# lucidrains/vector-quantize-pytorch

Hardware: NVIDIA H100
Metric: vectors quantized/sec at dim=256, codebook=1024; indices bit-exact vs ref (higher is better)
Workload: dtype bf16

## Files before the change

vector_quantize_pytorch_b200/csrc/ptx.cuh:

```cuda
#pragma once
#include <cuda.h>
#include <cuda_runtime.h>
#include <stdint.h>

namespace vqb {

__device__ __forceinline__ uint32_t smem_u32(const void* p) {
  return static_cast<uint32_t>(__cvta_generic_to_shared(p));
}

__device__ __forceinline__ void mbar_init(uint32_t bar, uint32_t count) {
  asm volatile("mbarrier.init.shared::cta.b64 [%0], %1;" ::"r"(bar), "r"(count));
}
__device__ __forceinline__ void fence_barrier_init() {
  asm volatile("fence.mbarrier_init.release.cluster;" ::: "memory");
}
__device__ __forceinline__ void mbar_arrive(uint32_t bar) {
  asm volatile("mbarrier.arrive.shared::cta.b64 _, [%0];" ::"r"(bar) : "memory");
}
__device__ __forceinline__ void mbar_arrive_expect_tx(uint32_t bar, uint32_t bytes) {
  asm volatile("mbarrier.arrive.expect_tx.shared::cta.b64 _, [%0], %1;" ::"r"(bar), "r"(bytes) : "memory");
}
__device__ __forceinline__ bool mbar_try_wait(uint32_t bar, uint32_t parity) {
  uint32_t ok;
  asm volatile(
      "{\n"
      ".reg .pred p;\n"
      "mbarrier.try_wait.parity.shared::cta.b64 p, [%1], %2;\n"
      "selp.u32 %0, 1, 0, p;\n"
      "}\n"
      : "=r"(ok)
      : "r"(bar), "r"(parity)
      : "memory");
  return ok != 0;
}

#ifndef VQB_WAIT_TIMEOUT_CYCLES
#define VQB_WAIT_TIMEOUT_CYCLES (8000000000ll)
#endif
__device__ __forceinline__ void mbar_wait(uint32_t bar, uint32_t parity) {
  if (mbar_try_wait(bar, parity)) return;
  const long long t0 = clock64();
  while (!mbar_try_wait(bar, parity)) {
    if (clock64() - t0 > VQB_WAIT_TIMEOUT_CYCLES) __trap();
  }
}

__device__ __forceinline__ void tma_prefetch_desc(const CUtensorMap* m) {
  asm volatile("prefetch.tensormap [%0];" ::"l"(reinterpret_cast<uint64_t>(m)) : "memory");
}
__device__ __forceinline__ void tma_load_3d(uint32_t dst, const CUtensorMap* m, uint32_t bar, int c0, int c1, int c2) {
  asm volatile(
      "cp.async.bulk.tensor.3d.shared::cluster.global.tile.mbarrier::complete_tx::bytes [%0], [%1, {%3, %4, %5}], [%2];"
      ::"r"(dst), "l"(reinterpret_cast<uint64_t>(m)), "r"(bar), "r"(c0), "r"(c1), "r"(c2)
      : "memory");
}

__device__ __forceinline__ void tma_prefetch_l2_3d(const CUtensorMap* m, int c0, int c1, int c2) {
  asm volatile("cp.async.bulk.prefetch.tensor.3d.L2.global.tile [%0, {%1, %2, %3}];"
               ::"l"(reinterpret_cast<uint64_t>(m)), "r"(c0), "r"(c1), "r"(c2)
               : "memory");
}

__device__ __forceinline__ uint64_t wgmma_desc_sw128(uint32_t saddr) {
  uint64_t d = 0;
  d |= static_cast<uint64_t>((saddr >> 4) & 0x3FFF);
  d |= static_cast<uint64_t>(1) << 16;
  d |= static_cast<uint64_t>(1024 >> 4) << 32;
  d |= static_cast<uint64_t>(1) << 62;
  return d;
}

__device__ __forceinline__ uint64_t wgmma_desc_sw32(uint32_t saddr) {
  uint64_t d = 0;
  d |= static_cast<uint64_t>((saddr >> 4) & 0x3FFF);
  d |= static_cast<uint64_t>(1) << 16;
  d |= static_cast<uint64_t>(256 >> 4) << 32;
  d |= static_cast<uint64_t>(3) << 62;
  return d;
}

__device__ __forceinline__ void fence_proxy_async_shared() { asm volatile("fence.proxy.async.shared::cta;" ::: "memory"); }
__device__ __forceinline__ void wgmma_fence() { asm volatile("wgmma.fence.sync.aligned;" ::: "memory"); }
__device__ __forceinline__ void wgmma_commit() { asm volatile("wgmma.commit_group.sync.aligned;" ::: "memory"); }
template <int N>
__device__ __forceinline__ void wgmma_wait() { asm volatile("wgmma.wait_group.sync.aligned %0;" ::"n"(N) : "memory"); }

template <int R>
__device__ __forceinline__ void fence_regs(float (&d)[R]) {
#pragma unroll
  for (int i = 0; i < R; ++i) asm volatile("" : "+f"(d[i])::"memory");
}

__device__ __forceinline__ void wgmma_m64n128k16_bf16(float (&d)[64], uint64_t adesc, uint64_t bdesc) {
  asm volatile(
      "{\n"
      "wgmma.mma_async.sync.aligned.m64n128k16.f32.bf16.bf16 "
      "{%0, %1, %2, %3, %4, %5, %6, %7, %8, %9, %10, %11, %12, %13, %14, %15, "
      "%16, %17, %18, %19, %20, %21, %22, %23, %24, %25, %26, %27, %28, %29, %30, %31, "
      "%32, %33, %34, %35, %36, %37, %38, %39, %40, %41, %42, %43, %44, %45, %46, %47, "
      "%48, %49, %50, %51, %52, %53, %54, %55, %56, %57, %58, %59, %60, %61, %62, %63}, "
      "%64, %65, 1, 1, 1, 0, 0;\n"
      "}\n"
      : "+f"(d[0]), "+f"(d[1]), "+f"(d[2]), "+f"(d[3]), "+f"(d[4]), "+f"(d[5]), "+f"(d[6]), "+f"(d[7]),
        "+f"(d[8]), "+f"(d[9]), "+f"(d[10]), "+f"(d[11]), "+f"(d[12]), "+f"(d[13]), "+f"(d[14]), "+f"(d[15]),
        "+f"(d[16]), "+f"(d[17]), "+f"(d[18]), "+f"(d[19]), "+f"(d[20]), "+f"(d[21]), "+f"(d[22]), "+f"(d[23]),
        "+f"(d[24]), "+f"(d[25]), "+f"(d[26]), "+f"(d[27]), "+f"(d[28]), "+f"(d[29]), "+f"(d[30]), "+f"(d[31]),
        "+f"(d[32]), "+f"(d[33]), "+f"(d[34]), "+f"(d[35]), "+f"(d[36]), "+f"(d[37]), "+f"(d[38]), "+f"(d[39]),
        "+f"(d[40]), "+f"(d[41]), "+f"(d[42]), "+f"(d[43]), "+f"(d[44]), "+f"(d[45]), "+f"(d[46]), "+f"(d[47]),
        "+f"(d[48]), "+f"(d[49]), "+f"(d[50]), "+f"(d[51]), "+f"(d[52]), "+f"(d[53]), "+f"(d[54]), "+f"(d[55]),
        "+f"(d[56]), "+f"(d[57]), "+f"(d[58]), "+f"(d[59]), "+f"(d[60]), "+f"(d[61]), "+f"(d[62]), "+f"(d[63])
      : "l"(adesc), "l"(bdesc));
}

__device__ __forceinline__ void wgmma_m64n128k16_bf16_rs_set(float (&d)[64], uint32_t a01, uint64_t bdesc) {
  asm volatile(
      "{\n"
      ".reg .pred p;\n"
      "setp.ne.b32 p, %67, 0;\n"
      "wgmma.mma_async.sync.aligned.m64n128k16.f32.bf16.bf16 "
      "{%0, %1, %2, %3, %4, %5, %6, %7, %8, %9, %10, %11, %12, %13, %14, %15, "
      "%16, %17, %18, %19, %20, %21, %22, %23, %24, %25, %26, %27, %28, %29, %30, %31, "
      "%32, %33, %34, %35, %36, %37, %38, %39, %40, %41, %42, %43, %44, %45, %46, %47, "
      "%48, %49, %50, %51, %52, %53, %54, %55, %56, %57, %58, %59, %60, %61, %62, %63}, "
      "{%64, %64, %65, %65}, %66, p, 1, 1, 0;\n"
      "}\n"
      : "=f"(d[0]), "=f"(d[1]), "=f"(d[2]), "=f"(d[3]), "=f"(d[4]), "=f"(d[5]), "=f"(d[6]), "=f"(d[7]),
        "=f"(d[8]), "=f"(d[9]), "=f"(d[10]), "=f"(d[11]), "=f"(d[12]), "=f"(d[13]), "=f"(d[14]), "=f"(d[15]),
        "=f"(d[16]), "=f"(d[17]), "=f"(d[18]), "=f"(d[19]), "=f"(d[20]), "=f"(d[21]), "=f"(d[22]), "=f"(d[23]),
        "=f"(d[24]), "=f"(d[25]), "=f"(d[26]), "=f"(d[27]), "=f"(d[28]), "=f"(d[29]), "=f"(d[30]), "=f"(d[31]),
        "=f"(d[32]), "=f"(d[33]), "=f"(d[34]), "=f"(d[35]), "=f"(d[36]), "=f"(d[37]), "=f"(d[38]), "=f"(d[39]),
        "=f"(d[40]), "=f"(d[41]), "=f"(d[42]), "=f"(d[43]), "=f"(d[44]), "=f"(d[45]), "=f"(d[46]), "=f"(d[47]),
        "=f"(d[48]), "=f"(d[49]), "=f"(d[50]), "=f"(d[51]), "=f"(d[52]), "=f"(d[53]), "=f"(d[54]), "=f"(d[55]),
        "=f"(d[56]), "=f"(d[57]), "=f"(d[58]), "=f"(d[59]), "=f"(d[60]), "=f"(d[61]), "=f"(d[62]), "=f"(d[63])
      : "r"(a01), "r"(0u), "l"(bdesc), "n"(0));
}

__device__ __forceinline__ void wgmma_m64n256k16_bf16(float (&d)[128], uint64_t adesc, uint64_t bdesc) {
  asm volatile(
      "{\n"
      "wgmma.mma_async.sync.aligned.m64n256k16.f32.bf16.bf16 "
      "{%0, %1, %2, %3, %4, %5, %6, %7, %8, %9, %10, %11, %12, %13, %14, %15, "
      "%16, %17, %18, %19, %20, %21, %22, %23, %24, %25, %26, %27, %28, %29, %30, %31, "
      "%32, %33, %34, %35, %36, %37, %38, %39, %40, %41, %42, %43, %44, %45, %46, %47, "
      "%48, %49, %50, %51, %52, %53, %54, %55, %56, %57, %58, %59, %60, %61, %62, %63, "
      "%64, %65, %66, %67, %68, %69, %70, %71, %72, %73, %74, %75, %76, %77, %78, %79, "
      "%80, %81, %82, %83, %84, %85, %86, %87, %88, %89, %90, %91, %92, %93, %94, %95, "
      "%96, %97, %98, %99, %100, %101, %102, %103, %104, %105, %106, %107, %108, %109, %110, %111, "
      "%112, %113, %114, %115, %116, %117, %118, %119, %120, %121, %122, %123, %124, %125, %126, %127}, "
      "%128, %129, 1, 1, 1, 0, 0;\n"
      "}\n"
      :
        "+f"(d[0]), "+f"(d[1]), "+f"(d[2]), "+f"(d[3]), "+f"(d[4]), "+f"(d[5]), "+f"(d[6]), "+f"(d[7]),
        "+f"(d[8]), "+f"(d[9]), "+f"(d[10]), "+f"(d[11]), "+f"(d[12]), "+f"(d[13]), "+f"(d[14]), "+f"(d[15]),
        "+f"(d[16]), "+f"(d[17]), "+f"(d[18]), "+f"(d[19]), "+f"(d[20]), "+f"(d[21]), "+f"(d[22]), "+f"(d[23]),
        "+f"(d[24]), "+f"(d[25]), "+f"(d[26]), "+f"(d[27]), "+f"(d[28]), "+f"(d[29]), "+f"(d[30]), "+f"(d[31]),
        "+f"(d[32]), "+f"(d[33]), "+f"(d[34]), "+f"(d[35]), "+f"(d[36]), "+f"(d[37]), "+f"(d[38]), "+f"(d[39]),
        "+f"(d[40]), "+f"(d[41]), "+f"(d[42]), "+f"(d[43]), "+f"(d[44]), "+f"(d[45]), "+f"(d[46]), "+f"(d[47]),
        "+f"(d[48]), "+f"(d[49]), "+f"(d[50]), "+f"(d[51]), "+f"(d[52]), "+f"(d[53]), "+f"(d[54]), "+f"(d[55]),
        "+f"(d[56]), "+f"(d[57]), "+f"(d[58]), "+f"(d[59]), "+f"(d[60]), "+f"(d[61]), "+f"(d[62]), "+f"(d[63]),
        "+f"(d[64]), "+f"(d[65]), "+f"(d[66]), "+f"(d[67]), "+f"(d[68]), "+f"(d[69]), "+f"(d[70]), "+f"(d[71]),
        "+f"(d[72]), "+f"(d[73]), "+f"(d[74]), "+f"(d[75]), "+f"(d[76]), "+f"(d[77]), "+f"(d[78]), "+f"(d[79]),
        "+f"(d[80]), "+f"(d[81]), "+f"(d[82]), "+f"(d[83]), "+f"(d[84]), "+f"(d[85]), "+f"(d[86]), "+f"(d[87]),
        "+f"(d[88]), "+f"(d[89]), "+f"(d[90]), "+f"(d[91]), "+f"(d[92]), "+f"(d[93]), "+f"(d[94]), "+f"(d[95]),
        "+f"(d[96]), "+f"(d[97]), "+f"(d[98]), "+f"(d[99]), "+f"(d[100]), "+f"(d[101]), "+f"(d[102]), "+f"(d[103]),
        "+f"(d[104]), "+f"(d[105]), "+f"(d[106]), "+f"(d[107]), "+f"(d[108]), "+f"(d[109]), "+f"(d[110]), "+f"(d[111]),
        "+f"(d[112]), "+f"(d[113]), "+f"(d[114]), "+f"(d[115]), "+f"(d[116]), "+f"(d[117]), "+f"(d[118]), "+f"(d[119]),
        "+f"(d[120]), "+f"(d[121]), "+f"(d[122]), "+f"(d[123]), "+f"(d[124]), "+f"(d[125]), "+f"(d[126]), "+f"(d[127])
      : "l"(adesc), "l"(bdesc));
}

__device__ __forceinline__ void wgmma_m64n256k16_bf16_ss_set(float (&d)[128], uint64_t adesc, uint64_t bdesc) {
  asm volatile(
      "{\n"
      ".reg .pred p;\n"
      "setp.ne.b32 p, %130, 0;\n"
      "wgmma.mma_async.sync.aligned.m64n256k16.f32.bf16.bf16 "
      "{%0, %1, %2, %3, %4, %5, %6, %7, %8, %9, %10, %11, %12, %13, %14, %15, "
      "%16, %17, %18, %19, %20, %21, %22, %23, %24, %25, %26, %27, %28, %29, %30, %31, "
      "%32, %33, %34, %35, %36, %37, %38, %39, %40, %41, %42, %43, %44, %45, %46, %47, "
      "%48, %49, %50, %51, %52, %53, %54, %55, %56, %57, %58, %59, %60, %61, %62, %63, "
      "%64, %65, %66, %67, %68, %69, %70, %71, %72, %73, %74, %75, %76, %77, %78, %79, "
      "%80, %81, %82, %83, %84, %85, %86, %87, %88, %89, %90, %91, %92, %93, %94, %95, "
      "%96, %97, %98, %99, %100, %101, %102, %103, %104, %105, %106, %107, %108, %109, %110, %111, "
      "%112, %113, %114, %115, %116, %117, %118, %119, %120, %121, %122, %123, %124, %125, %126, %127}, "
      "%128, %129, p, 1, 1, 0, 0;\n"
      "}\n"
      :
        "=f"(d[0]), "=f"(d[1]), "=f"(d[2]), "=f"(d[3]), "=f"(d[4]), "=f"(d[5]), "=f"(d[6]), "=f"(d[7]),
        "=f"(d[8]), "=f"(d[9]), "=f"(d[10]), "=f"(d[11]), "=f"(d[12]), "=f"(d[13]), "=f"(d[14]), "=f"(d[15]),
        "=f"(d[16]), "=f"(d[17]), "=f"(d[18]), "=f"(d[19]), "=f"(d[20]), "=f"(d[21]), "=f"(d[22]), "=f"(d[23]),
        "=f"(d[24]), "=f"(d[25]), "=f"(d[26]), "=f"(d[27]), "=f"(d[28]), "=f"(d[29]), "=f"(d[30]), "=f"(d[31]),
        "=f"(d[32]), "=f"(d[33]), "=f"(d[34]), "=f"(d[35]), "=f"(d[36]), "=f"(d[37]), "=f"(d[38]), "=f"(d[39]),
        "=f"(d[40]), "=f"(d[41]), "=f"(d[42]), "=f"(d[43]), "=f"(d[44]), "=f"(d[45]), "=f"(d[46]), "=f"(d[47]),
        "=f"(d[48]), "=f"(d[49]), "=f"(d[50]), "=f"(d[51]), "=f"(d[52]), "=f"(d[53]), "=f"(d[54]), "=f"(d[55]),
        "=f"(d[56]), "=f"(d[57]), "=f"(d[58]), "=f"(d[59]), "=f"(d[60]), "=f"(d[61]), "=f"(d[62]), "=f"(d[63]),
        "=f"(d[64]), "=f"(d[65]), "=f"(d[66]), "=f"(d[67]), "=f"(d[68]), "=f"(d[69]), "=f"(d[70]), "=f"(d[71]),
        "=f"(d[72]), "=f"(d[73]), "=f"(d[74]), "=f"(d[75]), "=f"(d[76]), "=f"(d[77]), "=f"(d[78]), "=f"(d[79]),
        "=f"(d[80]), "=f"(d[81]), "=f"(d[82]), "=f"(d[83]), "=f"(d[84]), "=f"(d[85]), "=f"(d[86]), "=f"(d[87]),
        "=f"(d[88]), "=f"(d[89]), "=f"(d[90]), "=f"(d[91]), "=f"(d[92]), "=f"(d[93]), "=f"(d[94]), "=f"(d[95]),
        "=f"(d[96]), "=f"(d[97]), "=f"(d[98]), "=f"(d[99]), "=f"(d[100]), "=f"(d[101]), "=f"(d[102]), "=f"(d[103]),
        "=f"(d[104]), "=f"(d[105]), "=f"(d[106]), "=f"(d[107]), "=f"(d[108]), "=f"(d[109]), "=f"(d[110]), "=f"(d[111]),
        "=f"(d[112]), "=f"(d[113]), "=f"(d[114]), "=f"(d[115]), "=f"(d[116]), "=f"(d[117]), "=f"(d[118]), "=f"(d[119]),
        "=f"(d[120]), "=f"(d[121]), "=f"(d[122]), "=f"(d[123]), "=f"(d[124]), "=f"(d[125]), "=f"(d[126]), "=f"(d[127])
      : "l"(adesc), "l"(bdesc), "n"(0));
}

__device__ __forceinline__ void wgmma_m64n256k16_bf16_rs_set(float (&d)[128], uint32_t a01, uint64_t bdesc) {
  asm volatile(
      "{\n"
      ".reg .pred p;\n"
      "setp.ne.b32 p, %131, 0;\n"
      "wgmma.mma_async.sync.aligned.m64n256k16.f32.bf16.bf16 "
      "{%0, %1, %2, %3, %4, %5, %6, %7, %8, %9, %10, %11, %12, %13, %14, %15, "
      "%16, %17, %18, %19, %20, %21, %22, %23, %24, %25, %26, %27, %28, %29, %30, %31, "
      "%32, %33, %34, %35, %36, %37, %38, %39, %40, %41, %42, %43, %44, %45, %46, %47, "
      "%48, %49, %50, %51, %52, %53, %54, %55, %56, %57, %58, %59, %60, %61, %62, %63, "
      "%64, %65, %66, %67, %68, %69, %70, %71, %72, %73, %74, %75, %76, %77, %78, %79, "
      "%80, %81, %82, %83, %84, %85, %86, %87, %88, %89, %90, %91, %92, %93, %94, %95, "
      "%96, %97, %98, %99, %100, %101, %102, %103, %104, %105, %106, %107, %108, %109, %110, %111, "
      "%112, %113, %114, %115, %116, %117, %118, %119, %120, %121, %122, %123, %124, %125, %126, %127}, "
      "{%128, %128, %129, %129}, %130, p, 1, 1, 0;\n"
      "}\n"
      :
        "=f"(d[0]), "=f"(d[1]), "=f"(d[2]), "=f"(d[3]), "=f"(d[4]), "=f"(d[5]), "=f"(d[6]), "=f"(d[7]),
        "=f"(d[8]), "=f"(d[9]), "=f"(d[10]), "=f"(d[11]), "=f"(d[12]), "=f"(d[13]), "=f"(d[14]), "=f"(d[15]),
        "=f"(d[16]), "=f"(d[17]), "=f"(d[18]), "=f"(d[19]), "=f"(d[20]), "=f"(d[21]), "=f"(d[22]), "=f"(d[23]),
        "=f"(d[24]), "=f"(d[25]), "=f"(d[26]), "=f"(d[27]), "=f"(d[28]), "=f"(d[29]), "=f"(d[30]), "=f"(d[31]),
        "=f"(d[32]), "=f"(d[33]), "=f"(d[34]), "=f"(d[35]), "=f"(d[36]), "=f"(d[37]), "=f"(d[38]), "=f"(d[39]),
        "=f"(d[40]), "=f"(d[41]), "=f"(d[42]), "=f"(d[43]), "=f"(d[44]), "=f"(d[45]), "=f"(d[46]), "=f"(d[47]),
        "=f"(d[48]), "=f"(d[49]), "=f"(d[50]), "=f"(d[51]), "=f"(d[52]), "=f"(d[53]), "=f"(d[54]), "=f"(d[55]),
        "=f"(d[56]), "=f"(d[57]), "=f"(d[58]), "=f"(d[59]), "=f"(d[60]), "=f"(d[61]), "=f"(d[62]), "=f"(d[63]),
        "=f"(d[64]), "=f"(d[65]), "=f"(d[66]), "=f"(d[67]), "=f"(d[68]), "=f"(d[69]), "=f"(d[70]), "=f"(d[71]),
        "=f"(d[72]), "=f"(d[73]), "=f"(d[74]), "=f"(d[75]), "=f"(d[76]), "=f"(d[77]), "=f"(d[78]), "=f"(d[79]),
        "=f"(d[80]), "=f"(d[81]), "=f"(d[82]), "=f"(d[83]), "=f"(d[84]), "=f"(d[85]), "=f"(d[86]), "=f"(d[87]),
        "=f"(d[88]), "=f"(d[89]), "=f"(d[90]), "=f"(d[91]), "=f"(d[92]), "=f"(d[93]), "=f"(d[94]), "=f"(d[95]),
        "=f"(d[96]), "=f"(d[97]), "=f"(d[98]), "=f"(d[99]), "=f"(d[100]), "=f"(d[101]), "=f"(d[102]), "=f"(d[103]),
        "=f"(d[104]), "=f"(d[105]), "=f"(d[106]), "=f"(d[107]), "=f"(d[108]), "=f"(d[109]), "=f"(d[110]), "=f"(d[111]),
        "=f"(d[112]), "=f"(d[113]), "=f"(d[114]), "=f"(d[115]), "=f"(d[116]), "=f"(d[117]), "=f"(d[118]), "=f"(d[119]),
        "=f"(d[120]), "=f"(d[121]), "=f"(d[122]), "=f"(d[123]), "=f"(d[124]), "=f"(d[125]), "=f"(d[126]), "=f"(d[127])
      : "r"(a01), "r"(0u), "l"(bdesc), "n"(0));
}

}
```

vector_quantize_pytorch_b200/csrc/vq_assign.cu:

```cuda
#include <type_traits>
#include "ptx.cuh"
#include "vqb_common.cuh"
#include "gather_row.cuh"
#include "epilogue.cuh"

#ifdef VQB_PROFILE
#define PROF_CLOCK() clock64()
#else
#define PROF_CLOCK() 0ll
#endif

namespace vqb {

constexpr int BM = 128;
constexpr int WM = 64;
constexpr int BN_STAGE = 128;
constexpr int BK = 64;
constexpr int A_SUB_BYTES = BM * BK * 2;
constexpr int B_SUB_BYTES = BN_STAGE * BK * 2;
constexpr int MAX_A_SUB = 8;
constexpr int MAX_STAGES = 8;
constexpr int NUM_CONSUMER_WARPS = 8;
constexpr int NUM_STORE_WARPS = 3;
constexpr int NUM_THREADS = 128 + NUM_CONSUMER_WARPS * 32;
constexpr int SMEM_CTRL_BYTES = 14336;
constexpr int SMEM_LIMIT = 232448;
constexpr int SEED_BYTES = BN_STAGE * 32;

struct AssignParams {
  int64_t N;
  int D, K, Kpad;
  int n_a, n_passes;
  int KB;
  int n_stages;
  int n_seed;
  int stream_a;
  const uint16_t* a_global;
  const uint16_t* bext;
  int num_row_tiles, num_code_steps;
  float margin_rel;
  const float* cmax;
  int32_t* idx;
  int32_t* idx_prov;
  int32_t* hist;
  int hist_shift;
  vqb_flag_entry* flagged;
  int32_t* flag_count;
  float* dbg_best;
  const uint8_t* row_mask;
  long long* prof;
  FusedOut fo;
  int copy_mode;
  int resid_mode;
  int metric;
  const uint16_t* b_hi;
  const float* cnorm2;
  uint32_t tagmask, mul1, mulm1;
};

struct Ctrl {
  uint64_t a_full[MAX_A_SUB], a_empty[MAX_A_SUB];
  uint64_t b_full[MAX_STAGES], b_empty[MAX_STAGES];
  uint64_t g_full[2], g_empty[2];
  int gidx[2][BM];
  MergeSlot merge[BM][3];
  float x2[BM];
};
static_assert(sizeof(Ctrl) <= SMEM_CTRL_BYTES, "control block too large");

template <int GB>
__device__ __forceinline__ float tail_rows(const FusedOut& fo, const int64_t (&rows)[GB], const int (&ks)[GB], int D, int lane) {
  if (fo.dtype == VQB_DTYPE_BF16) return gather_rows<VQB_DTYPE_BF16, GB>(fo, rows, ks, D, lane);
  return gather_rows<VQB_DTYPE_F32, GB>(fo, rows, ks, D, lane);
}

__device__ __forceinline__ float sq_diff16(const uint4& xa, const uint4& ca, bool bf) {
  const uint32_t xw[4] = {xa.x, xa.y, xa.z, xa.w}, cw[4] = {ca.x, ca.y, ca.z, ca.w};
  float s = 0.f;
#pragma unroll
  for (int e = 0; e < 4; ++e) {
    if (bf) {
      const float d0 = __uint_as_float(xw[e] << 16) - __uint_as_float(cw[e] << 16);
      const float d1 = __uint_as_float(xw[e] & 0xFFFF0000u) - __uint_as_float(cw[e] & 0xFFFF0000u);
      s += bf16_round(d0 * d0);
      s += bf16_round(d1 * d1);
    } else {
      const float d = __uint_as_float(xw[e]) - __uint_as_float(cw[e]);
      s += d * d;
    }
  }
  return s;
}

template <int WN>
struct StepLocals {
  float loss_ = 0.f;
  __device__ __forceinline__ float& loss() { return loss_; }
};
template <>
struct StepLocals<256> {
  static __device__ __forceinline__ float& loss() {
    __shared__ float s[NUM_CONSUMER_WARPS * 32];
    return s[threadIdx.x - 128];
  }
  static __device__ __forceinline__ uint32_t* bias_ones() {
    __shared__ __align__(256) uint32_t o[WM * 16 / 2];
    return o;
  }
  __device__ __forceinline__ StepLocals() { loss() = 0.f; }
};
constexpr int WIDE_STATIC_SMEM = NUM_CONSUMER_WARPS * 32 * 4 + WM * 16 * 2;

template <int TAIL, int WN>
__global__ void __launch_bounds__(NUM_THREADS, 1)
vq_assign_kernel(const __grid_constant__ CUtensorMap tmA, const __grid_constant__ CUtensorMap tmB,
                 const __grid_constant__ CUtensorMap tmS, const AssignParams p) {
  static_assert(WN == 128 || WN == 256, "code step width");
  constexpr int SPAN = WN / BN_STAGE;
  constexpr uint32_t STEP_SEED_BYTES = SPAN * SEED_BYTES;
  extern __shared__ __align__(1024) uint8_t smem[];
  Ctrl* ctrl = reinterpret_cast<Ctrl*>(smem);
  const uint32_t smem_base = smem_u32(smem);
  const uint32_t a_base = (smem_base + SMEM_CTRL_BYTES + 1023u) & ~1023u;
  const bool stream_a = WN == 128 && p.stream_a;
  const int n_sub = stream_a ? 0 : p.n_a * p.KB;
  const uint32_t b_base = a_base + n_sub * A_SUB_BYTES;
  const uint32_t a_stage_bytes = stream_a ? A_SUB_BYTES : 0;
  const uint32_t stage_stride = a_stage_bytes + SPAN * B_SUB_BYTES;
  const int n_ring = p.n_stages / SPAN;
  const uint32_t seed_base = b_base + n_ring * stage_stride;

  const int warp = threadIdx.x >> 5;
  const int lane = threadIdx.x & 31;

  if (threadIdx.x == 0) {
    tma_prefetch_desc(&tmA);
    tma_prefetch_desc(&tmB);
    tma_prefetch_desc(&tmS);
    for (int s = 0; s < n_sub; ++s) {
      mbar_init(smem_u32(&ctrl->a_full[s]), 1);
      mbar_init(smem_u32(&ctrl->a_empty[s]), NUM_CONSUMER_WARPS);
    }
    for (int s = 0; s < n_ring; ++s) {
      mbar_init(smem_u32(&ctrl->b_full[s]), 1);
      mbar_init(smem_u32(&ctrl->b_empty[s]), NUM_CONSUMER_WARPS);
    }
    for (int s = 0; s < 2; ++s) {
      mbar_init(smem_u32(&ctrl->g_full[s]), NUM_CONSUMER_WARPS);
      mbar_init(smem_u32(&ctrl->g_empty[s]), NUM_STORE_WARPS);
    }
    fence_barrier_init();
  }
  if constexpr (WN == 256) {
    for (int i = threadIdx.x; i < WM * 16 / 2; i += NUM_THREADS) StepLocals<256>::bias_ones()[i] = 0x3F803F80u;
    fence_proxy_async_shared();
  }
  __syncthreads();

  if (warp == 0) {
    if (lane == 0) {
      long long w_empty = 0, w_aempty = 0;
      const long long pstart = PROF_CLOCK();
      int stage = 0, gstep = 0;
      uint32_t ph = 0;
      for (int t = 0, tile = static_cast<int>(blockIdx.x); tile < p.num_row_tiles; ++t, tile += static_cast<int>(gridDim.x)) {
        const int row0 = tile * BM;
        if (!stream_a && tile + static_cast<int>(gridDim.x) < p.num_row_tiles) {
          for (int ap = 0; ap < p.n_a; ++ap)
            for (int kb = 0; kb < p.KB; ++kb) tma_prefetch_l2_3d(&tmA, kb * BK, row0 + static_cast<int>(gridDim.x) * BM, ap);
        }
        for (int ct = 0; ct < p.num_code_steps; ++ct, ++gstep) {
          for (int kb = 0; kb < p.KB; ++kb) {
            for (int ps = 0; ps < p.n_passes; ++ps) {
              const int bplane = (ps == 1) ? 1 : 0;
              const int aplane = (ps == 2) ? 1 : 0;
              if (!stream_a && ct == 0 && (ps == 0 || ps == 2)) {
                const int sub = aplane * p.KB + kb;
                { const long long c0 = PROF_CLOCK(); mbar_wait(smem_u32(&ctrl->a_empty[sub]), (t & 1) ^ 1); w_aempty += PROF_CLOCK() - c0; }
                mbar_arrive_expect_tx(smem_u32(&ctrl->a_full[sub]), A_SUB_BYTES);
                tma_load_3d(a_base + sub * A_SUB_BYTES, &tmA, smem_u32(&ctrl->a_full[sub]), kb * BK, row0, aplane);
              }
              { const long long c0 = PROF_CLOCK(); mbar_wait(smem_u32(&ctrl->b_empty[stage]), ph ^ 1); w_empty += PROF_CLOCK() - c0; }
              const bool seeds = kb == 0 && ps == 0;
              mbar_arrive_expect_tx(smem_u32(&ctrl->b_full[stage]), stage_stride + (seeds ? STEP_SEED_BYTES : 0));
              if (seeds)
                tma_load_3d(seed_base + (gstep % p.n_seed) * STEP_SEED_BYTES, &tmS, smem_u32(&ctrl->b_full[stage]), 0, ct * WN, 0);
              if (stream_a)
                tma_load_3d(b_base + stage * stage_stride, &tmA, smem_u32(&ctrl->b_full[stage]), kb * BK, row0, aplane);
              tma_load_3d(b_base + stage * stage_stride + a_stage_bytes, &tmB, smem_u32(&ctrl->b_full[stage]), kb * BK,
                          ct * WN, bplane);
              if (++stage == n_ring) { stage = 0; ph ^= 1; }
            }
          }
        }
      }
      if (p.prof) {
        p.prof[blockIdx.x * 16 + 0] = w_empty;
        p.prof[blockIdx.x * 16 + 1] = PROF_CLOCK() - pstart;
        p.prof[blockIdx.x * 16 + 6] = w_aempty;
      }
    }
  } else if (warp <= NUM_STORE_WARPS) {
    const int sw = warp - 1;
    float lsum = 0.f;
    for (int t = 0, tile = static_cast<int>(blockIdx.x); p.fo.enabled && tile < p.num_row_tiles; ++t, tile += static_cast<int>(gridDim.x)) {
      mbar_wait(smem_u32(&ctrl->g_full[t & 1]), (t >> 1) & 1);
      const int* gi = ctrl->gidx[t & 1];
      if (TAIL >= 1) {
        constexpr int CB = 4;
        const bool bf = p.fo.dtype == VQB_DTYPE_BF16;
        const int row_bytes = p.D * (bf ? 2 : 4);
        const uint8_t* src = bf ? reinterpret_cast<const uint8_t*>(p.b_hi) : reinterpret_cast<const uint8_t*>(p.fo.embed);
        const uint8_t* xin = static_cast<const uint8_t*>(p.fo.x_eff);
        uint8_t* dst = static_cast<uint8_t*>(TAIL == 2 ? p.fo.resid_out : p.fo.q_out);
        for (int r0 = sw * CB; r0 < BM; r0 += NUM_STORE_WARPS * CB) {
          int ks[CB];
          bool ex[CB];
#pragma unroll
          for (int b = 0; b < CB; ++b) {
            const int g = gi[r0 + b];
            ex[b] = g < -1;
            ks[b] = ex[b] ? -2 - g : g;
          }
          const int64_t row_base = static_cast<int64_t>(tile) * BM + r0;
          if (p.fo.idx64_out && lane < CB && ks[lane & (CB - 1)] >= 0) {
            int kk = 0;
#pragma unroll
            for (int b = 0; b < CB; ++b) kk = (lane == b) ? ks[b] : kk;
            p.fo.idx64_out[(row_base + lane) * p.fo.idx_stride] = kk;
          }
          if (dst || (ex[0] | ex[1] | ex[2] | ex[3])) {
            for (int off = lane * 16; off < row_bytes; off += 512) {
              uint4 v[CB];
#pragma unroll
              for (int b = 0; b < CB; ++b)
                if (ks[b] >= 0) v[b] = __ldg(reinterpret_cast<const uint4*>(src + static_cast<int64_t>(ks[b]) * row_bytes + off));
              if (TAIL == 1) {
#pragma unroll
                for (int b = 0; b < CB; ++b)
                  if (ex[b]) lsum += sq_diff16(*reinterpret_cast<const uint4*>(xin + (row_base + b) * row_bytes + off), v[b], bf);
              }
              if (TAIL == 2) {
                uint4 x[CB];
#pragma unroll
                for (int b = 0; b < CB; ++b)
                  if (ks[b] >= 0) x[b] = *reinterpret_cast<const uint4*>(xin + (row_base + b) * row_bytes + off);
#pragma unroll
                for (int b = 0; b < CB; ++b) {
                  if (ks[b] < 0) continue;
                  if (ex[b]) lsum += sq_diff16(x[b], v[b], bf);
                  const uint32_t xw[4] = {x[b].x, x[b].y, x[b].z, x[b].w}, cw[4] = {v[b].x, v[b].y, v[b].z, v[b].w};
                  uint32_t rw[4];
                  if (bf) {
#pragma unroll
                    for (int e = 0; e < 4; ++e) {
                      const float d0 = __uint_as_float(xw[e] << 16) - __uint_as_float(cw[e] << 16);
                      const float d1 = __uint_as_float(xw[e] & 0xFFFF0000u) - __uint_as_float(cw[e] & 0xFFFF0000u);
                      asm("cvt.rn.bf16x2.f32 %0, %1, %2;" : "=r"(rw[e]) : "f"(d1), "f"(d0));
                    }
                  } else {
#pragma unroll
                    for (int e = 0; e < 4; ++e) rw[e] = __float_as_uint(__uint_as_float(xw[e]) - __uint_as_float(cw[e]));
                    if (p.fo.planes_out) {
                      const float rf[4] = {__uint_as_float(rw[0]), __uint_as_float(rw[1]), __uint_as_float(rw[2]), __uint_as_float(rw[3])};
                      store_planes4(p.fo.planes_out, p.fo.planes_stride, ((row_base + b) * row_bytes + off) >> 2, rf);
                    }
                  }
                  v[b] = make_uint4(rw[0], rw[1], rw[2], rw[3]);
                }
              }
#pragma unroll
              for (int b = 0; b < CB; ++b)
                if (dst && ks[b] >= 0) *reinterpret_cast<uint4*>(dst + (row_base + b) * row_bytes + off) = v[b];
            }
          }
        }
      } else {
        constexpr int GB = 2;
        for (int r0 = sw * GB; r0 < BM; r0 += NUM_STORE_WARPS * GB) {
          int64_t rows[GB];
          int ks[GB];
          bool any = false;
#pragma unroll
          for (int b = 0; b < GB; ++b) {
            ks[b] = gi[r0 + b];
            rows[b] = ks[b] >= 0 ? static_cast<int64_t>(tile) * BM + r0 + b : -1;
            any |= ks[b] >= 0;
          }
          if (!any) continue;
          lsum += tail_rows<GB>(p.fo, rows, ks, p.D, lane);
        }
      }
      __syncwarp();
      if (lane == 0) mbar_arrive(smem_u32(&ctrl->g_empty[t & 1]));
    }
    if (p.fo.enabled && p.fo.loss_sum) {
      const double w = warp_sum(static_cast<double>(lsum));
      if (lane == 0) atomicAdd(p.fo.loss_sum, w);
    }
  } else {
    const int wg = (warp >> 2) - 1;
    const int q = lane & 3;
    const int rit0 = wg * WM + (warp & 3) * 16 + (lane >> 2);
    const int n_items = p.KB * p.n_passes;
    const uint32_t a_row_off = wg * WM * 128;
    const uint32_t bias_a = q == 0 ? 0x3F803F80u : (q == 1 ? 0x00003F80u : 0u);
    long long w_full = 0, w_afull = 0, w_gap = 0, gap0 = -1;
    const long long cstart = PROF_CLOCK();
    float acc[WN / 2];
    int stage = 0, gstep = 0;
    uint32_t ph = 0;
    StepLocals<WN> locals;
    auto release = [&](int st, int sub) {
      if (lane == 0) {
        mbar_arrive(smem_u32(&ctrl->b_empty[st]));
        if (sub >= 0) mbar_arrive(smem_u32(&ctrl->a_empty[sub]));
      }
    };
    auto row_norms = [&](int tile, float (&xlo)[2]) {
#pragma unroll
      for (int h = 0; h < 2; ++h) {
        const int64_t row = static_cast<int64_t>(tile) * BM + rit0 + 8 * h;
        float a = 0.f, alo = 0.f;
        if (row < p.N) {
          const uint16_t* hp = p.a_global + row * p.D;
          for (int c = q * 8; c < p.D; c += 32) {
            const uint4 u = __ldg(reinterpret_cast<const uint4*>(hp + c));
            uint4 l = make_uint4(0u, 0u, 0u, 0u);
            if (p.n_a == 2) l = __ldg(reinterpret_cast<const uint4*>(hp + p.N * p.D + c));
            const uint32_t w[4] = {u.x, u.y, u.z, u.w};
            const uint32_t wl[4] = {l.x, l.y, l.z, l.w};
#pragma unroll
            for (int e = 0; e < 4; ++e) {
              const float h0 = __uint_as_float(w[e] << 16), h1 = __uint_as_float(w[e] & 0xFFFF0000u);
              const float l0 = __uint_as_float(wl[e] << 16), l1 = __uint_as_float(wl[e] & 0xFFFF0000u);
              a = fmaf(h0 + l0, h0 + l0, a);
              a = fmaf(h1 + l1, h1 + l1, a);
              alo = fmaf(l0, l0, alo);
              alo = fmaf(l1, l1, alo);
            }
          }
        }
        a += __shfl_xor_sync(0xffffffffu, a, 1);
        a += __shfl_xor_sync(0xffffffffu, a, 2);
        alo += __shfl_xor_sync(0xffffffffu, alo, 1);
        alo += __shfl_xor_sync(0xffffffffu, alo, 2);
        if (q == 0) ctrl->x2[rit0 + 8 * h] = a;
        xlo[h] = alo;
      }
    };
    auto init_band = [&](auto (&sc)[2], float (&xlo)[2]) {
      const bool euclid = p.metric != VQB_METRIC_COSINE;
      const float cmax = __ldg(p.cmax + CMAX_NORM);
      const float cres = __ldg(p.cmax + CMAX_RES);
      const float caux = p.n_a == 2 ? 0x1.02p-8f * cmax + __ldg(p.cmax + CMAX_LO) : 0.f;
      __syncwarp();
#pragma unroll
      for (int h = 0; h < 2; ++h) {
        const float x2 = ctrl->x2[rit0 + 8 * h];
        const float xn = sqrtf(x2);
        const float xc = xn * cmax;
        xlo[h] = p.n_a == 2 ? sqrtf(xlo[h]) * 1.0001f : 0.f;
        sc[h].init(2.f * (xn * cres + xlo[h] * caux + p.margin_rel * xc + (euclid ? 0x1p-21f * cmax * cmax : 0.f)) +
                   0x1p-18f * (xc + (euclid ? 0.5f * cmax * cmax : 0.f)) +
                   (euclid ? 0x1p-22f * (x2 + cmax * cmax) + 1e-8f : 1e-30f));
      }
    };
    for (int t = 0, tile = static_cast<int>(blockIdx.x); tile < p.num_row_tiles; ++t, tile += static_cast<int>(gridDim.x)) {
      typename std::conditional<WN == 128, ScanReg, ScanState<16>>::type sc[2];
      ScanQueue<16> sq[2];

      float xlo[2] = {0.f, 0.f};
      for (int ct = 0; ct < p.num_code_steps; ++ct) {
        const bool last_ct = ct == p.num_code_steps - 1;
        if (WN == 256 && ct == 0) {
          row_norms(tile, xlo);
          init_band(sc, xlo);
        }
        if (gap0 >= 0) w_gap += PROF_CLOCK() - gap0;
        { const long long c0 = PROF_CLOCK(); mbar_wait(smem_u32(&ctrl->b_full[stage]), ph); w_full += PROF_CLOCK() - c0; }
        wgmma_fence();
        const uint64_t sd = wgmma_desc_sw32(seed_base + (gstep % p.n_seed) * STEP_SEED_BYTES);
        if constexpr (WN == 128) wgmma_m64n128k16_bf16_rs_set(acc, bias_a, sd);
        else wgmma_m64n256k16_bf16_ss_set(acc, wgmma_desc_sw32(smem_u32(StepLocals<256>::bias_ones())), sd);
        int kb = 0, ps = 0;
        int pend_stage = -1, pend_sub = -1;
        for (int i = 0; i < n_items; ++i) {
          const int aplane = (ps == 2) ? 1 : 0;
          const int sub = aplane * p.KB + kb;
          if (ct == 0 && !stream_a) { const long long c0 = PROF_CLOCK(); mbar_wait(smem_u32(&ctrl->a_full[sub]), t & 1); w_afull += PROF_CLOCK() - c0; }
          if (i > 0) { const long long c0 = PROF_CLOCK(); mbar_wait(smem_u32(&ctrl->b_full[stage]), ph); w_full += PROF_CLOCK() - c0; }
          const uint32_t st_addr = b_base + stage * stage_stride;
          const uint32_t a_addr = (stream_a ? st_addr : a_base + sub * A_SUB_BYTES) + a_row_off;
          const uint64_t ad = wgmma_desc_sw128(a_addr);
          const uint64_t bd = wgmma_desc_sw128(st_addr + a_stage_bytes);
          fence_regs(acc);
          wgmma_fence();
#pragma unroll
          for (int k = 0; k < 8; k += 2) {
            if constexpr (WN == 128) wgmma_m64n128k16_bf16(acc, ad + k, bd + k);
            else wgmma_m64n256k16_bf16(acc, ad + k, bd + k);
          }
          wgmma_commit();
          if (i == n_items - 1) gap0 = PROF_CLOCK();
          wgmma_wait<1>();
          fence_regs(acc);
          if (pend_stage >= 0) release(pend_stage, pend_sub);
          const bool last_use = last_ct && !stream_a && (aplane == 1 ? ps == 2 : ps == 1);
          pend_stage = stage;
          pend_sub = last_use ? sub : -1;
          if (++stage == n_ring) { stage = 0; ph ^= 1; }
          if (++ps == p.n_passes) { ps = 0; ++kb; }
        }
        if (WN == 128 && ct == 0) row_norms(tile, xlo);
        wgmma_wait<0>();
        fence_regs(acc);
        release(pend_stage, pend_sub);
        ++gstep;
        if ((ct + 1) * WN > p.Kpad) {
#pragma unroll
          for (int j = 0; j < WN / 8; ++j)
#pragma unroll
            for (int b = 0; b < 2; ++b)
              if (ct * WN + 8 * j + 2 * q + b >= p.Kpad) { acc[4 * j + b] = -3.0e38f; acc[4 * j + 2 + b] = -3.0e38f; }
        }

        if (WN == 128 && ct == 0) {
          init_band(sc, xlo);
        } else if (ct > 0) {
#pragma unroll
          for (int h = 0; h < 2; ++h) {
            float m = sc[h].t1;
            m = fmaxf(m, __shfl_xor_sync(0xffffffffu, m, 1));
            m = fmaxf(m, __shfl_xor_sync(0xffffffffu, m, 2));
            sc[h].raise(m);
          }
        }
#pragma unroll
        for (int g = 0; g < WN / 64; ++g) {
#pragma unroll
          for (int h = 0; h < 2; ++h) {
            uint32_t r[16];
#pragma unroll
            for (int e = 0; e < 16; ++e) r[e] = __float_as_uint(acc[4 * (8 * g + (e >> 1)) + 2 * h + (e & 1)]);
            if constexpr (WN == 128) sc[h].template scan16<true, false>(sq[h], r, ct * WN + 64 * g + 2 * q, p.mul1);
            else sc[h].template scan16<true>(sq[h], r, ct * WN + 64 * g + 2 * q);
          }
        }
      }

      if (p.fo.enabled) mbar_wait(smem_u32(&ctrl->g_empty[t & 1]), ((t >> 1) & 1) ^ 1);
#pragma unroll
      for (int h = 0; h < 2; ++h) {
        const int rit = rit0 + 8 * h;
        RowState st;
        sc[h].finish(sq[h], st, p.tagmask, p.mul1, p.mulm1);
        MergeSlot* slots = ctrl->merge[rit];
        if (q != 0) publish(&slots[q - 1], st);
        __syncwarp();
        if (q == 0) {
          const RowResult rr = merge_slices(st, slots, 3, 1);
          const int n = rr.n, i0 = rr.i0, i1 = rr.i1;
          const float best = rr.best;
          const int64_t row = static_cast<int64_t>(tile) * BM + rit;
          const bool live = row < p.N && (p.row_mask == nullptr || __ldg(p.row_mask + row) != 0);
          bool exact_loss = false;
          if (TAIL >= 1 && p.fo.loss_sum && live && n < 2) {
            float d2 = ctrl->x2[rit] - 2.f * best;
            if (p.metric == VQB_METRIC_COSINE) d2 += __ldg(p.cnorm2 + i0);
            exact_loss = !(d2 >= 0x1p14f * st.W);
            if (!exact_loss) locals.loss() += d2;
          }
          if (p.fo.enabled) ctrl->gidx[t & 1][rit] = (live && n < 2) ? (exact_loss ? -2 - i0 : i0) : -1;
          if (row < p.N && !live) {
            p.idx[row] = -1;
            if (p.idx_prov) p.idx_prov[row] = -1;
          } else if (row < p.N) {
            p.idx[row] = i0;
            if (p.idx_prov) p.idx_prov[row] = (n < 2) ? i0 : -1;
            if (p.hist && n < 2) atomicAdd(p.hist + static_cast<size_t>(tile >> p.hist_shift) * p.K + i0, 1);
            if (p.dbg_best) p.dbg_best[row] = best;
            if (n >= 2) {
              const bool many = n > 3;
              const int s = many ? static_cast<int>(p.N) - 1 - atomicAdd(p.flag_count + 1, 1) : atomicAdd(p.flag_count, 1);
              vqb_flag_entry e;
              e.row = static_cast<int32_t>(row);
              e.cand0 = many ? 0 : i0;
              e.cand1 = many ? 0 : i1;
              e.cand2 = rr.i2;
              e.count = n;
              e.pad[0] = e.pad[1] = e.pad[2] = 0;
              p.flagged[s] = e;
            }
          }
        }
        __syncwarp();
      }
      if (p.fo.enabled && lane == 0) mbar_arrive(smem_u32(&ctrl->g_full[t & 1]));
    }
    if (TAIL >= 1 && p.fo.loss_sum) {
      const double w = warp_sum(static_cast<double>(locals.loss()));
      if (lane == 0) atomicAdd(p.fo.loss_sum, w);
    }
    if (p.prof && threadIdx.x == 128) {
      p.prof[blockIdx.x * 16 + 2] = w_full;
      p.prof[blockIdx.x * 16 + 3] = PROF_CLOCK() - cstart;
      p.prof[blockIdx.x * 16 + 4] = w_gap;
      p.prof[blockIdx.x * 16 + 5] = w_afull;
    }
  }
}

typedef CUresult (*PFN_encodeTiled)(CUtensorMap*, CUtensorMapDataType, cuuint32_t, void*, const cuuint64_t*,
                                    const cuuint64_t*, const cuuint32_t*, const cuuint32_t*, CUtensorMapInterleave,
                                    CUtensorMapSwizzle, CUtensorMapL2promotion, CUtensorMapFloatOOBfill);

static PFN_encodeTiled get_encode_fn() {
  static PFN_encodeTiled fn = nullptr;
  static bool tried = false;
  if (!tried) {
    tried = true;
    void* f = nullptr;
    cudaDriverEntryPointQueryResult qres;
    if (cudaGetDriverEntryPoint("cuTensorMapEncodeTiled", &f, cudaEnableDefault, &qres) == cudaSuccess &&
        qres == cudaDriverEntryPointSuccess)
      fn = reinterpret_cast<PFN_encodeTiled>(f);
  }
  return fn;
}

static int make_map(CUtensorMap* m, const void* base, int cols, int64_t rows, int planes, int box_cols, int box_rows,
                    CUtensorMapSwizzle swz) {
  PFN_encodeTiled enc = get_encode_fn();
  if (!enc) return VQB_E_DRIVER;
  cuuint64_t dims[3] = {static_cast<cuuint64_t>(cols), static_cast<cuuint64_t>(rows), static_cast<cuuint64_t>(planes)};
  cuuint64_t strides[2] = {static_cast<cuuint64_t>(cols) * 2, static_cast<cuuint64_t>(cols) * 2 * static_cast<cuuint64_t>(rows)};
  cuuint32_t box[3] = {static_cast<cuuint32_t>(box_cols), static_cast<cuuint32_t>(box_rows), 1};
  cuuint32_t estr[3] = {1, 1, 1};
  CUresult r = enc(m, CU_TENSOR_MAP_DATA_TYPE_BFLOAT16, 3, const_cast<void*>(base), dims, strides, box, estr,
                   CU_TENSOR_MAP_INTERLEAVE_NONE, swz, CU_TENSOR_MAP_L2_PROMOTION_L2_256B, CU_TENSOR_MAP_FLOAT_OOB_FILL_NONE);
  return r == CUDA_SUCCESS ? VQB_OK : VQB_E_DRIVER;
}

struct AssignPlan {
  int stream_a, n_stages, n_seed, n_items, KB, smem_bytes;
};

static int assign_plan(int n_a, int D, int n_passes, AssignPlan* pl) {
  if (D <= 0 || (n_a != 1 && n_a != 2)) return VQB_E_INVALID;
  if (n_passes == 0) n_passes = n_a + 1;
  if (n_passes != n_a + 1) return VQB_E_UNSUPPORTED;
  if (D % 8 != 0) return VQB_E_UNSUPPORTED;
  const int KB = (D + BK - 1) / BK;
  const int stream_a = n_a * KB > MAX_A_SUB ? 1 : 0;
  const int a_bytes = stream_a ? 0 : n_a * KB * A_SUB_BYTES;
  const int stage_bytes = B_SUB_BYTES + (stream_a ? A_SUB_BYTES : 0);
  const int fixed = SMEM_CTRL_BYTES + 1024  + a_bytes;
  const int n_items = KB * n_passes;
  int stages = MAX_STAGES;
  auto seed_slots = [&](int st) { return (st + n_items - 1) / n_items; };
  while (stages >= 2 && fixed + stages * stage_bytes + seed_slots(stages) * SEED_BYTES > SMEM_LIMIT) --stages;
  if (stages < 2) return VQB_E_UNSUPPORTED;
  pl->stream_a = stream_a;
  pl->n_stages = stages;
  pl->n_seed = seed_slots(stages);
  pl->n_items = n_items;
  pl->KB = KB;
  pl->smem_bytes = fixed + stages * stage_bytes + pl->n_seed * SEED_BYTES;
  return VQB_OK;
}

static bool wide_step(const AssignPlan& pl, int Kpad, int* n_seed, int* smem_bytes) {
  if (pl.stream_a || pl.n_stages % 2 != 0 || Kpad <= BN_STAGE) return false;
  const int ring = pl.n_stages / 2;
  const int seeds = (ring + pl.n_items - 1) / pl.n_items;
  const int bytes = pl.smem_bytes - pl.n_seed * SEED_BYTES + seeds * 2 * SEED_BYTES;
  if (bytes + WIDE_STATIC_SMEM > SMEM_LIMIT) return false;
  *n_seed = seeds;
  *smem_bytes = bytes;
  return true;
}

}

using namespace vqb;

extern "C" int vqb_debug_assign_plan(int n_a, int D, int n_passes, int* out6) {
  if (!out6) return VQB_E_INVALID;
  AssignPlan pl;
  const int rc = assign_plan(n_a, D, n_passes, &pl);
  if (rc) return rc;
  out6[0] = pl.stream_a; out6[1] = pl.n_stages; out6[2] = pl.n_seed;
  out6[3] = pl.n_items; out6[4] = pl.KB; out6[5] = pl.smem_bytes;
  return VQB_OK;
}

extern "C" int vqb_padded_codes(int K) {
  if (K <= 0) return 0;
  const int BN = code_tile(K);
  return (K + BN - 1) / BN * BN;
}

static long long* g_prof = nullptr;
static int g_dbg_mode = 0;
extern "C" int vqb_debug_set_mode(int mode) { g_dbg_mode = mode; return VQB_OK; }
extern "C" int vqb_debug_active(void) { return (g_prof != nullptr) || (g_dbg_mode != 0); }
extern "C" int vqb_debug_set_profile_buffer(void* buf) { g_prof = static_cast<long long*>(buf); return VQB_OK; }

extern "C" int vqb_assign(const void* a_planes, int n_a, int64_t N, int D, const void* b_planes, const void* bext,
                          const float* cmax, int K, float margin_rel, int n_passes, int32_t* idx,
                          vqb_flag_entry* flagged, int32_t* flag_count, float* dbg_best,
                          const vqb_fused_outputs* fused, void* stream) {
  return vqb_assign_ex(a_planes, n_a, N, D, b_planes, bext, cmax, K, margin_rel, n_passes, idx, flagged, flag_count,
                       dbg_best, fused, VQB_METRIC_EUCLID, nullptr, stream);
}

extern "C" int vqb_assign_ex(const void* a_planes, int n_a, int64_t N, int D, const void* b_planes, const void* bext,
                             const float* cmax, int K, float margin_rel, int n_passes, int32_t* idx,
                             vqb_flag_entry* flagged, int32_t* flag_count, float* dbg_best,
                             const vqb_fused_outputs* fused, int metric, const float* cnorm2, void* stream) {
  return vqb::assign_launch(a_planes, n_a, N, D, b_planes, bext, cmax, K, margin_rel, n_passes, idx, nullptr, nullptr, 0,
                            flagged, flag_count, dbg_best, fused, metric, cnorm2, stream);
}

int vqb::assign_launch(const void* a_planes, int n_a, int64_t N, int D, const void* b_planes, const void* bext,
                       const float* cmax, int K, float margin_rel, int n_passes, int32_t* idx, int32_t* idx_prov,
                       int32_t* hist, int hist_shift, vqb_flag_entry* flagged, int32_t* flag_count, float* dbg_best,
                       const vqb_fused_outputs* fused, int metric, const float* cnorm2, void* stream, const uint8_t* row_mask) {
  if (!a_planes || !b_planes || !bext || !cmax || !idx || !flagged || !flag_count) return VQB_E_INVALID;
  if (N <= 0 || K <= 0) return VQB_E_INVALID;
  AssignPlan plan;
  int rc = assign_plan(n_a, D, n_passes, &plan);
  if (rc) return rc;
  if (n_passes == 0) n_passes = n_a + 1;
  if (N > (static_cast<int64_t>(1) << 31) - BM) return VQB_E_UNSUPPORTED;
  if ((reinterpret_cast<uintptr_t>(a_planes) | reinterpret_cast<uintptr_t>(b_planes) | reinterpret_cast<uintptr_t>(bext)) & 15)
    return VQB_E_ALIGN;
  AssignParams p;
  rc = make_fused(&p.fo, fused, D, N);
  if (rc) return rc;
  rc = check_device();
  if (rc) return rc;

  p.N = N; p.D = D; p.K = K;
  p.Kpad = vqb_padded_codes(K);
  p.n_a = n_a; p.n_passes = n_passes; p.KB = plan.KB;
  p.num_row_tiles = static_cast<int>((N + BM - 1) / BM);
  int smem_bytes = plan.smem_bytes;
  p.n_seed = plan.n_seed;
  const bool wide = wide_step(plan, p.Kpad, &p.n_seed, &smem_bytes);
  const int WN = wide ? 256 : 128;
  p.num_code_steps = (p.Kpad + WN - 1) / WN;
  p.margin_rel = margin_rel;
  p.cmax = cmax; p.idx = idx; p.idx_prov = idx_prov; p.hist = hist; p.hist_shift = hist_shift; p.flagged = flagged; p.flag_count = flag_count; p.dbg_best = dbg_best;
  p.row_mask = row_mask;
  p.prof = g_prof;
  p.tagmask = 0xFFFFFFF0u; p.mul1 = 1u; p.mulm1 = 0xFFFFFFFFu;
  p.metric = metric;
  p.cnorm2 = cnorm2;
  p.b_hi = static_cast<const uint16_t*>(b_planes);
  p.bext = static_cast<const uint16_t*>(bext);
  p.copy_mode = p.fo.enabled && !p.fo.resid_out && !(metric == VQB_METRIC_COSINE && p.fo.loss_sum && !cnorm2);
  p.resid_mode = p.fo.enabled && p.fo.resid_out && !p.fo.q_out &&
                 (!p.fo.x_raw || p.fo.x_raw == p.fo.x_eff) && !(metric == VQB_METRIC_COSINE && p.fo.loss_sum && !cnorm2);
  p.stream_a = plan.stream_a;
  p.a_global = static_cast<const uint16_t*>(a_planes);
  p.n_stages = plan.n_stages;

  CUtensorMap tmA, tmB, tmS;
  rc = make_map(&tmA, a_planes, D, N, n_a, BK, BM, CU_TENSOR_MAP_SWIZZLE_128B);
  if (rc) return rc;
  rc = make_map(&tmB, b_planes, D, p.Kpad, 2, BK, WN, CU_TENSOR_MAP_SWIZZLE_128B);
  if (rc) return rc;
  rc = make_map(&tmS, bext, 16, p.Kpad, 1, 16, WN, CU_TENSOR_MAP_SWIZZLE_32B);
  if (rc) return rc;

  static bool attr_set = false;
  if (!attr_set) {
    void (*const kernels[6])(CUtensorMap, CUtensorMap, CUtensorMap, AssignParams) = {
        vq_assign_kernel<0, 128>, vq_assign_kernel<1, 128>, vq_assign_kernel<2, 128>,
        vq_assign_kernel<0, 256>, vq_assign_kernel<1, 256>, vq_assign_kernel<2, 256>};
    for (int i = 0; i < 6; ++i) {
      const int dyn = i < 3 ? SMEM_LIMIT : SMEM_LIMIT - WIDE_STATIC_SMEM;
      const cudaError_t e = cudaFuncSetAttribute(kernels[i], cudaFuncAttributeMaxDynamicSharedMemorySize, dyn);
      if (e != cudaSuccess) return static_cast<int>(e);
    }
    attr_set = true;
  }
  const int grid = p.num_row_tiles < num_sms() ? p.num_row_tiles : num_sms();
  cudaStream_t s = static_cast<cudaStream_t>(stream);
  if (wide) {
    if (p.copy_mode) vq_assign_kernel<1, 256><<<grid, NUM_THREADS, smem_bytes, s>>>(tmA, tmB, tmS, p);
    else if (p.resid_mode) vq_assign_kernel<2, 256><<<grid, NUM_THREADS, smem_bytes, s>>>(tmA, tmB, tmS, p);
    else vq_assign_kernel<0, 256><<<grid, NUM_THREADS, smem_bytes, s>>>(tmA, tmB, tmS, p);
  } else {
    if (p.copy_mode) vq_assign_kernel<1, 128><<<grid, NUM_THREADS, smem_bytes, s>>>(tmA, tmB, tmS, p);
    else if (p.resid_mode) vq_assign_kernel<2, 128><<<grid, NUM_THREADS, smem_bytes, s>>>(tmA, tmB, tmS, p);
    else vq_assign_kernel<0, 128><<<grid, NUM_THREADS, smem_bytes, s>>>(tmA, tmB, tmS, p);
  }
  return static_cast<int>(cudaGetLastError());
}
```

Before: 379.6 million.

## Replace wide 256-code step with ping-pong accumulators overlapping scan and WGMMA

Drops the single m64n256 wide-step path in favor of two m64n128 accumulator sets. The scan/argmin of one code block runs while the tensor-core MMAs for the next block are in flight. Row norms for the next tile are now computed ahead of time by the store warps into double-buffered shared memory and signalled through a new mbarrier, taking that work off the consumer critical path. The cost is more register pressure from two accumulator arrays, extra shared memory, and added synchronization complexity. Shape constraints also tighten: Kpad must be a multiple of two stages.

```diff
diff --git a/vector_quantize_pytorch_b200/csrc/ptx.cuh b/vector_quantize_pytorch_b200/csrc/ptx.cuh
--- a/vector_quantize_pytorch_b200/csrc/ptx.cuh
+++ b/vector_quantize_pytorch_b200/csrc/ptx.cuh
@@ -136,110 +136,27 @@
       : "r"(a01), "r"(0u), "l"(bdesc), "n"(0));
 }
 
-__device__ __forceinline__ void wgmma_m64n256k16_bf16(float (&d)[128], uint64_t adesc, uint64_t bdesc) {
+__device__ __forceinline__ void wgmma_m64n128k16_bf16_ss_set(float (&d)[64], uint64_t adesc, uint64_t bdesc) {
   asm volatile(
       "{\n"
-      "wgmma.mma_async.sync.aligned.m64n256k16.f32.bf16.bf16 "
+      ".reg .pred p;\n"
+      "setp.ne.b32 p, %66, 0;\n"
+      "wgmma.mma_async.sync.aligned.m64n128k16.f32.bf16.bf16 "
       "{%0, %1, %2, %3, %4, %5, %6, %7, %8, %9, %10, %11, %12, %13, %14, %15, "
       "%16, %17, %18, %19, %20, %21, %22, %23, %24, %25, %26, %27, %28, %29, %30, %31, "
       "%32, %33, %34, %35, %36, %37, %38, %39, %40, %41, %42, %43, %44, %45, %46, %47, "
-      "%48, %49, %50, %51, %52, %53, %54, %55, %56, %57, %58, %59, %60, %61, %62, %63, "
-      "%64, %65, %66, %67, %68, %69, %70, %71, %72, %73, %74, %75, %76, %77, %78, %79, "
-      "%80, %81, %82, %83, %84, %85, %86, %87, %88, %89, %90, %91, %92, %93, %94, %95, "
-      "%96, %97, %98, %99, %100, %101, %102, %103, %104, %105, %106, %107, %108, %109, %110, %111, "
-      "%112, %113, %114, %115, %116, %117, %118, %119, %120, %121, %122, %123, %124, %125, %126, %127}, "
-      "%128, %129, 1, 1, 1, 0, 0;\n"
+      "%48, %49, %50, %51, %52, %53, %54, %55, %56, %57, %58, %59, %60, %61, %62, %63}, "
+      "%64, %65, p, 1, 1, 0, 0;\n"
       "}\n"
-      :
-        "+f"(d[0]), "+f"(d[1]), "+f"(d[2]), "+f"(d[3]), "+f"(d[4]), "+f"(d[5]), "+f"(d[6]), "+f"(d[7]),
-        "+f"(d[8]), "+f"(d[9]), "+f"(d[10]), "+f"(d[11]), "+f"(d[12]), "+f"(d[13]), "+f"(d[14]), "+f"(d[15]),
-        "+f"(d[16]), "+f"(d[17]), "+f"(d[18]), "+f"(d[19]), "+f"(d[20]), "+f"(d[21]), "+f"(d[22]), "+f"(d[23]),
-        "+f"(d[24]), "+f"(d[25]), "+f"(d[26]), "+f"(d[27]), "+f"(d[28]), "+f"(d[29]), "+f"(d[30]), "+f"(d[31]),
-        "+f"(d[32]), "+f"(d[33]), "+f"(d[34]), "+f"(d[35]), "+f"(d[36]), "+f"(d[37]), "+f"(d[38]), "+f"(d[39]),
-        "+f"(d[40]), "+f"(d[41]), "+f"(d[42]), "+f"(d[43]), "+f"(d[44]), "+f"(d[45]), "+f"(d[46]), "+f"(d[47]),
-        "+f"(d[48]), "+f"(d[49]), "+f"(d[50]), "+f"(d[51]), "+f"(d[52]), "+f"(d[53]), "+f"(d[54]), "+f"(d[55]),
-        "+f"(d[56]), "+f"(d[57]), "+f"(d[58]), "+f"(d[59]), "+f"(d[60]), "+f"(d[61]), "+f"(d[62]), "+f"(d[63]),
-        "+f"(d[64]), "+f"(d[65]), "+f"(d[66]), "+f"(d[67]), "+f"(d[68]), "+f"(d[69]), "+f"(d[70]), "+f"(d[71]),
-        "+f"(d[72]), "+f"(d[73]), "+f"(d[74]), "+f"(d[75]), "+f"(d[76]), "+f"(d[77]), "+f"(d[78]), "+f"(d[79]),
-        "+f"(d[80]), "+f"(d[81]), "+f"(d[82]), "+f"(d[83]), "+f"(d[84]), "+f"(d[85]), "+f"(d[86]), "+f"(d[87]),
-        "+f"(d[88]), "+f"(d[89]), "+f"(d[90]), "+f"(d[91]), "+f"(d[92]), "+f"(d[93]), "+f"(d[94]), "+f"(d[95]),
-        "+f"(d[96]), "+f"(d[97]), "+f"(d[98]), "+f"(d[99]), "+f"(d[100]), "+f"(d[101]), "+f"(d[102]), "+f"(d[103]),
-        "+f"(d[104]), "+f"(d[105]), "+f"(d[106]), "+f"(d[107]), "+f"(d[108]), "+f"(d[109]), "+f"(d[110]), "+f"(d[111]),
-        "+f"(d[112]), "+f"(d[113]), "+f"(d[114]), "+f"(d[115]), "+f"(d[116]), "+f"(d[117]), "+f"(d[118]), "+f"(d[119]),
-        "+f"(d[120]), "+f"(d[121]), "+f"(d[122]), "+f"(d[123]), "+f"(d[124]), "+f"(d[125]), "+f"(d[126]), "+f"(d[127])
-      : "l"(adesc), "l"(bdesc));
-}
-
-__device__ __forceinline__ void wgmma_m64n256k16_bf16_ss_set(float (&d)[128], uint64_t adesc, uint64_t bdesc) {
-  asm volatile(
-      "{\n"
-      ".reg .pred p;\n"
-      "setp.ne.b32 p, %130, 0;\n"
-      "wgmma.mma_async.sync.aligned.m64n256k16.f32.bf16.bf16 "
-      "{%0, %1, %2, %3, %4, %5, %6, %7, %8, %9, %10, %11, %12, %13, %14, %15, "
-      "%16, %17, %18, %19, %20, %21, %22, %23, %24, %25, %26, %27, %28, %29, %30, %31, "
-      "%32, %33, %34, %35, %36, %37, %38, %39, %40, %41, %42, %43, %44, %45, %46, %47, "
-      "%48, %49, %50, %51, %52, %53, %54, %55, %56, %57, %58, %59, %60, %61, %62, %63, "
-      "%64, %65, %66, %67, %68, %69, %70, %71, %72, %73, %74, %75, %76, %77, %78, %79, "
-      "%80, %81, %82, %83, %84, %85, %86, %87, %88, %89, %90, %91, %92, %93, %94, %95, "
-      "%96, %97, %98, %99, %100, %101, %102, %103, %104, %105, %106, %107, %108, %109, %110, %111, "
-      "%112, %113, %114, %115, %116, %117, %118, %119, %120, %121, %122, %123, %124, %125, %126, %127}, "
-      "%128, %129, p, 1, 1, 0, 0;\n"
-      "}\n"
-      :
-        "=f"(d[0]), "=f"(d[1]), "=f"(d[2]), "=f"(d[3]), "=f"(d[4]), "=f"(d[5]), "=f"(d[6]), "=f"(d[7]),
+      : "=f"(d[0]), "=f"(d[1]), "=f"(d[2]), "=f"(d[3]), "=f"(d[4]), "=f"(d[5]), "=f"(d[6]), "=f"(d[7]),
         "=f"(d[8]), "=f"(d[9]), "=f"(d[10]), "=f"(d[11]), "=f"(d[12]), "=f"(d[13]), "=f"(d[14]), "=f"(d[15]),
         "=f"(d[16]), "=f"(d[17]), "=f"(d[18]), "=f"(d[19]), "=f"(d[20]), "=f"(d[21]), "=f"(d[22]), "=f"(d[23]),
         "=f"(d[24]), "=f"(d[25]), "=f"(d[26]), "=f"(d[27]), "=f"(d[28]), "=f"(d[29]), "=f"(d[30]), "=f"(d[31]),
         "=f"(d[32]), "=f"(d[33]), "=f"(d[34]), "=f"(d[35]), "=f"(d[36]), "=f"(d[37]), "=f"(d[38]), "=f"(d[39]),
         "=f"(d[40]), "=f"(d[41]), "=f"(d[42]), "=f"(d[43]), "=f"(d[44]), "=f"(d[45]), "=f"(d[46]), "=f"(d[47]),
         "=f"(d[48]), "=f"(d[49]), "=f"(d[50]), "=f"(d[51]), "=f"(d[52]), "=f"(d[53]), "=f"(d[54]), "=f"(d[55]),
-        "=f"(d[56]), "=f"(d[57]), "=f"(d[58]), "=f"(d[59]), "=f"(d[60]), "=f"(d[61]), "=f"(d[62]), "=f"(d[63]),
-        "=f"(d[64]), "=f"(d[65]), "=f"(d[66]), "=f"(d[67]), "=f"(d[68]), "=f"(d[69]), "=f"(d[70]), "=f"(d[71]),
-        "=f"(d[72]), "=f"(d[73]), "=f"(d[74]), "=f"(d[75]), "=f"(d[76]), "=f"(d[77]), "=f"(d[78]), "=f"(d[79]),
-        "=f"(d[80]), "=f"(d[81]), "=f"(d[82]), "=f"(d[83]), "=f"(d[84]), "=f"(d[85]), "=f"(d[86]), "=f"(d[87]),
-        "=f"(d[88]), "=f"(d[89]), "=f"(d[90]), "=f"(d[91]), "=f"(d[92]), "=f"(d[93]), "=f"(d[94]), "=f"(d[95]),
-        "=f"(d[96]), "=f"(d[97]), "=f"(d[98]), "=f"(d[99]), "=f"(d[100]), "=f"(d[101]), "=f"(d[102]), "=f"(d[103]),
-        "=f"(d[104]), "=f"(d[105]), "=f"(d[106]), "=f"(d[107]), "=f"(d[108]), "=f"(d[109]), "=f"(d[110]), "=f"(d[111]),
-        "=f"(d[112]), "=f"(d[113]), "=f"(d[114]), "=f"(d[115]), "=f"(d[116]), "=f"(d[117]), "=f"(d[118]), "=f"(d[119]),
-        "=f"(d[120]), "=f"(d[121]), "=f"(d[122]), "=f"(d[123]), "=f"(d[124]), "=f"(d[125]), "=f"(d[126]), "=f"(d[127])
+        "=f"(d[56]), "=f"(d[57]), "=f"(d[58]), "=f"(d[59]), "=f"(d[60]), "=f"(d[61]), "=f"(d[62]), "=f"(d[63])
       : "l"(adesc), "l"(bdesc), "n"(0));
 }
 
-__device__ __forceinline__ void wgmma_m64n256k16_bf16_rs_set(float (&d)[128], uint32_t a01, uint64_t bdesc) {
-  asm volatile(
-      "{\n"
-      ".reg .pred p;\n"
-      "setp.ne.b32 p, %131, 0;\n"
-      "wgmma.mma_async.sync.aligned.m64n256k16.f32.bf16.bf16 "
-      "{%0, %1, %2, %3, %4, %5, %6, %7, %8, %9, %10, %11, %12, %13, %14, %15, "
-      "%16, %17, %18, %19, %20, %21, %22, %23, %24, %25, %26, %27, %28, %29, %30, %31, "
-      "%32, %33, %34, %35, %36, %37, %38, %39, %40, %41, %42, %43, %44, %45, %46, %47, "
-      "%48, %49, %50, %51, %52, %53, %54, %55, %56, %57, %58, %59, %60, %61, %62, %63, "
-      "%64, %65, %66, %67, %68, %69, %70, %71, %72, %73, %74, %75, %76, %77, %78, %79, "
-      "%80, %81, %82, %83, %84, %85, %86, %87, %88, %89, %90, %91, %92, %93, %94, %95, "
-      "%96, %97, %98, %99, %100, %101, %102, %103, %104, %105, %106, %107, %108, %109, %110, %111, "
-      "%112, %113, %114, %115, %116, %117, %118, %119, %120, %121, %122, %123, %124, %125, %126, %127}, "
-      "{%128, %128, %129, %129}, %130, p, 1, 1, 0;\n"
-      "}\n"
-      :
-        "=f"(d[0]), "=f"(d[1]), "=f"(d[2]), "=f"(d[3]), "=f"(d[4]), "=f"(d[5]), "=f"(d[6]), "=f"(d[7]),
-        "=f"(d[8]), "=f"(d[9]), "=f"(d[10]), "=f"(d[11]), "=f"(d[12]), "=f"(d[13]), "=f"(d[14]), "=f"(d[15]),
-        "=f"(d[16]), "=f"(d[17]), "=f"(d[18]), "=f"(d[19]), "=f"(d[20]), "=f"(d[21]), "=f"(d[22]), "=f"(d[23]),
-        "=f"(d[24]), "=f"(d[25]), "=f"(d[26]), "=f"(d[27]), "=f"(d[28]), "=f"(d[29]), "=f"(d[30]), "=f"(d[31]),
-        "=f"(d[32]), "=f"(d[33]), "=f"(d[34]), "=f"(d[35]), "=f"(d[36]), "=f"(d[37]), "=f"(d[38]), "=f"(d[39]),
-        "=f"(d[40]), "=f"(d[41]), "=f"(d[42]), "=f"(d[43]), "=f"(d[44]), "=f"(d[45]), "=f"(d[46]), "=f"(d[47]),
-        "=f"(d[48]), "=f"(d[49]), "=f"(d[50]), "=f"(d[51]), "=f"(d[52]), "=f"(d[53]), "=f"(d[54]), "=f"(d[55]),
-        "=f"(d[56]), "=f"(d[57]), "=f"(d[58]), "=f"(d[59]), "=f"(d[60]), "=f"(d[61]), "=f"(d[62]), "=f"(d[63]),
-        "=f"(d[64]), "=f"(d[65]), "=f"(d[66]), "=f"(d[67]), "=f"(d[68]), "=f"(d[69]), "=f"(d[70]), "=f"(d[71]),
-        "=f"(d[72]), "=f"(d[73]), "=f"(d[74]), "=f"(d[75]), "=f"(d[76]), "=f"(d[77]), "=f"(d[78]), "=f"(d[79]),
-        "=f"(d[80]), "=f"(d[81]), "=f"(d[82]), "=f"(d[83]), "=f"(d[84]), "=f"(d[85]), "=f"(d[86]), "=f"(d[87]),
-        "=f"(d[88]), "=f"(d[89]), "=f"(d[90]), "=f"(d[91]), "=f"(d[92]), "=f"(d[93]), "=f"(d[94]), "=f"(d[95]),
-        "=f"(d[96]), "=f"(d[97]), "=f"(d[98]), "=f"(d[99]), "=f"(d[100]), "=f"(d[101]), "=f"(d[102]), "=f"(d[103]),
-        "=f"(d[104]), "=f"(d[105]), "=f"(d[106]), "=f"(d[107]), "=f"(d[108]), "=f"(d[109]), "=f"(d[110]), "=f"(d[111]),
-        "=f"(d[112]), "=f"(d[113]), "=f"(d[114]), "=f"(d[115]), "=f"(d[116]), "=f"(d[117]), "=f"(d[118]), "=f"(d[119]),
-        "=f"(d[120]), "=f"(d[121]), "=f"(d[122]), "=f"(d[123]), "=f"(d[124]), "=f"(d[125]), "=f"(d[126]), "=f"(d[127])
-      : "r"(a01), "r"(0u), "l"(bdesc), "n"(0));
 }
-
-}
diff --git a/vector_quantize_pytorch_b200/csrc/vq_assign.cu b/vector_quantize_pytorch_b200/csrc/vq_assign.cu
--- a/vector_quantize_pytorch_b200/csrc/vq_assign.cu
+++ b/vector_quantize_pytorch_b200/csrc/vq_assign.cu
@@ -62,6 +62,7 @@
   uint64_t a_full[MAX_A_SUB], a_empty[MAX_A_SUB];
   uint64_t b_full[MAX_STAGES], b_empty[MAX_STAGES];
   uint64_t g_full[2], g_empty[2];
+  uint64_t n_full[2];
   int gidx[2][BM];
   MergeSlot merge[BM][3];
   float x2[BM];
@@ -92,13 +93,13 @@
   return s;
 }
 
-template <int WN>
+template <bool PIPE>
 struct StepLocals {
   float loss_ = 0.f;
   __device__ __forceinline__ float& loss() { return loss_; }
 };
 template <>
-struct StepLocals<256> {
+struct StepLocals<true> {
   static __device__ __forceinline__ float& loss() {
     __shared__ float s[NUM_CONSUMER_WARPS * 32];
     return s[threadIdx.x - 128];
@@ -107,27 +108,57 @@
     __shared__ __align__(256) uint32_t o[WM * 16 / 2];
     return o;
   }
+  static __device__ __forceinline__ float* norms(int b) {
+    __shared__ float n[2][2 * BM];
+    return n[b];
+  }
   __device__ __forceinline__ StepLocals() { loss() = 0.f; }
 };
-constexpr int WIDE_STATIC_SMEM = NUM_CONSUMER_WARPS * 32 * 4 + WM * 16 * 2;
-
-template <int TAIL, int WN>
+constexpr int PIPE_STATIC_SMEM = NUM_CONSUMER_WARPS * 32 * 4 + WM * 16 * 2 + 2 * 2 * BM * 4;
+
+__device__ __forceinline__ void quad_row_norms(const AssignParams& p, int64_t row, int q, float& a, float& alo) {
+  a = 0.f;
+  alo = 0.f;
+  if (row < p.N) {
+    const uint16_t* hp = p.a_global + row * p.D;
+    for (int c = q * 8; c < p.D; c += 32) {
+      const uint4 u = __ldg(reinterpret_cast<const uint4*>(hp + c));
+      uint4 l = make_uint4(0u, 0u, 0u, 0u);
+      if (p.n_a == 2) l = __ldg(reinterpret_cast<const uint4*>(hp + p.N * p.D + c));
+      const uint32_t w[4] = {u.x, u.y, u.z, u.w};
+      const uint32_t wl[4] = {l.x, l.y, l.z, l.w};
+#pragma unroll
+      for (int e = 0; e < 4; ++e) {
+        const float h0 = __uint_as_float(w[e] << 16), h1 = __uint_as_float(w[e] & 0xFFFF0000u);
+        const float l0 = __uint_as_float(wl[e] << 16), l1 = __uint_as_float(wl[e] & 0xFFFF0000u);
+        a = fmaf(h0 + l0, h0 + l0, a);
+        a = fmaf(h1 + l1, h1 + l1, a);
+        alo = fmaf(l0, l0, alo);
+        alo = fmaf(l1, l1, alo);
+      }
+    }
+  }
+  a += __shfl_xor_sync(0xffffffffu, a, 1);
+  a += __shfl_xor_sync(0xffffffffu, a, 2);
+  alo += __shfl_xor_sync(0xffffffffu, alo, 1);
+  alo += __shfl_xor_sync(0xffffffffu, alo, 2);
+}
+
+template <int TAIL, bool PIPE>
 __global__ void __launch_bounds__(NUM_THREADS, 1)
 vq_assign_kernel(const __grid_constant__ CUtensorMap tmA, const __grid_constant__ CUtensorMap tmB,
                  const __grid_constant__ CUtensorMap tmS, const AssignParams p) {
-  static_assert(WN == 128 || WN == 256, "code step width");
-  constexpr int SPAN = WN / BN_STAGE;
-  constexpr uint32_t STEP_SEED_BYTES = SPAN * SEED_BYTES;
+  constexpr int WN = BN_STAGE;
   extern __shared__ __align__(1024) uint8_t smem[];
   Ctrl* ctrl = reinterpret_cast<Ctrl*>(smem);
   const uint32_t smem_base = smem_u32(smem);
   const uint32_t a_base = (smem_base + SMEM_CTRL_BYTES + 1023u) & ~1023u;
-  const bool stream_a = WN == 128 && p.stream_a;
+  const bool stream_a = !PIPE && p.stream_a;
   const int n_sub = stream_a ? 0 : p.n_a * p.KB;
   const uint32_t b_base = a_base + n_sub * A_SUB_BYTES;
   const uint32_t a_stage_bytes = stream_a ? A_SUB_BYTES : 0;
-  const uint32_t stage_stride = a_stage_bytes + SPAN * B_SUB_BYTES;
-  const int n_ring = p.n_stages / SPAN;
+  const uint32_t stage_stride = a_stage_bytes + B_SUB_BYTES;
+  const int n_ring = p.n_stages;
   const uint32_t seed_base = b_base + n_ring * stage_stride;
 
   const int warp = threadIdx.x >> 5;
@@ -148,11 +179,12 @@
     for (int s = 0; s < 2; ++s) {
       mbar_init(smem_u32(&ctrl->g_full[s]), NUM_CONSUMER_WARPS);
       mbar_init(smem_u32(&ctrl->g_empty[s]), NUM_STORE_WARPS);
+      mbar_init(smem_u32(&ctrl->n_full[s]), NUM_STORE_WARPS);
     }
     fence_barrier_init();
   }
-  if constexpr (WN == 256) {
-    for (int i = threadIdx.x; i < WM * 16 / 2; i += NUM_THREADS) StepLocals<256>::bias_ones()[i] = 0x3F803F80u;
+  if constexpr (PIPE) {
+    for (int i = threadIdx.x; i < WM * 16 / 2; i += NUM_THREADS) StepLocals<true>::bias_ones()[i] = 0x3F803F80u;
     fence_proxy_async_shared();
   }
   __syncthreads();
@@ -182,9 +214,9 @@
               }
               { const long long c0 = PROF_CLOCK(); mbar_wait(smem_u32(&ctrl->b_empty[stage]), ph ^ 1); w_empty += PROF_CLOCK() - c0; }
               const bool seeds = kb == 0 && ps == 0;
-              mbar_arrive_expect_tx(smem_u32(&ctrl->b_full[stage]), stage_stride + (seeds ? STEP_SEED_BYTES : 0));
+              mbar_arrive_expect_tx(smem_u32(&ctrl->b_full[stage]), stage_stride + (seeds ? SEED_BYTES : 0));
               if (seeds)
-                tma_load_3d(seed_base + (gstep % p.n_seed) * STEP_SEED_BYTES, &tmS, smem_u32(&ctrl->b_full[stage]), 0, ct * WN, 0);
+                tma_load_3d(seed_base + (gstep % p.n_seed) * SEED_BYTES, &tmS, smem_u32(&ctrl->b_full[stage]), 0, ct * WN, 0);
               if (stream_a)
                 tma_load_3d(b_base + stage * stage_stride, &tmA, smem_u32(&ctrl->b_full[stage]), kb * BK, row0, aplane);
               tma_load_3d(b_base + stage * stage_stride + a_stage_bytes, &tmB, smem_u32(&ctrl->b_full[stage]), kb * BK,
@@ -203,10 +235,26 @@
   } else if (warp <= NUM_STORE_WARPS) {
     const int sw = warp - 1;
     float lsum = 0.f;
-    for (int t = 0, tile = static_cast<int>(blockIdx.x); p.fo.enabled && tile < p.num_row_tiles; ++t, tile += static_cast<int>(gridDim.x)) {
+    auto tile_norms = [&](int tile, int b) {
+      float* nb = StepLocals<true>::norms(b);
+      for (int r0 = sw * 8; r0 < BM; r0 += NUM_STORE_WARPS * 8) {
+        const int r = r0 + (lane >> 2);
+        float a, alo;
+        quad_row_norms(p, static_cast<int64_t>(tile) * BM + r, lane & 3, a, alo);
+        if ((lane & 3) == 0) { nb[r] = a; nb[BM + r] = alo; }
+      }
+      __syncwarp();
+      if (lane == 0) mbar_arrive(smem_u32(&ctrl->n_full[b]));
+    };
+    for (int t = 0, tile = static_cast<int>(blockIdx.x); (PIPE || p.fo.enabled) && tile < p.num_row_tiles; ++t, tile += static_cast<int>(gridDim.x)) {
+      if constexpr (PIPE) {
+        if (t == 0) tile_norms(tile, 0);
+        if (tile + static_cast<int>(gridDim.x) < p.num_row_tiles) tile_norms(tile + static_cast<int>(gridDim.x), (t + 1) & 1);
+      }
       mbar_wait(smem_u32(&ctrl->g_full[t & 1]), (t >> 1) & 1);
       const int* gi = ctrl->gidx[t & 1];
-      if (TAIL >= 1) {
+      if (!p.fo.enabled) {
+      } else if (TAIL >= 1) {
         constexpr int CB = 4;
         const bool bf = p.fo.dtype == VQB_DTYPE_BF16;
         const int row_bytes = p.D * (bf ? 2 : 4);
@@ -302,15 +350,14 @@
     const int wg = (warp >> 2) - 1;
     const int q = lane & 3;
     const int rit0 = wg * WM + (warp & 3) * 16 + (lane >> 2);
-    const int n_items = p.KB * p.n_passes;
     const uint32_t a_row_off = wg * WM * 128;
     const uint32_t bias_a = q == 0 ? 0x3F803F80u : (q == 1 ? 0x00003F80u : 0u);
-    long long w_full = 0, w_afull = 0, w_gap = 0, gap0 = -1;
+    long long w_full = 0, w_afull = 0, w_gap = 0, gap0 = -1, w_tile = 0, w_merge = 0, w_gempty = 0;
     const long long cstart = PROF_CLOCK();
-    float acc[WN / 2];
-    int stage = 0, gstep = 0;
+    float accA[64], accB[64];
+    int stage = 0, gstep = 0, kb = 0, ps = 0, pend_stage = -1, pend_sub = -1;
     uint32_t ph = 0;
-    StepLocals<WN> locals;
+    StepLocals<PIPE> locals;
     auto release = [&](int st, int sub) {
       if (lane == 0) {
         mbar_arrive(smem_u32(&ctrl->b_empty[st]));
@@ -320,36 +367,13 @@
     auto row_norms = [&](int tile, float (&xlo)[2]) {
 #pragma unroll
       for (int h = 0; h < 2; ++h) {
-        const int64_t row = static_cast<int64_t>(tile) * BM + rit0 + 8 * h;
-        float a = 0.f, alo = 0.f;
-        if (row < p.N) {
-          const uint16_t* hp = p.a_global + row * p.D;
-          for (int c = q * 8; c < p.D; c += 32) {
-            const uint4 u = __ldg(reinterpret_cast<const uint4*>(hp + c));
-            uint4 l = make_uint4(0u, 0u, 0u, 0u);
-            if (p.n_a == 2) l = __ldg(reinterpret_cast<const uint4*>(hp + p.N * p.D + c));
-            const uint32_t w[4] = {u.x, u.y, u.z, u.w};
-            const uint32_t wl[4] = {l.x, l.y, l.z, l.w};
-#pragma unroll
-            for (int e = 0; e < 4; ++e) {
-              const float h0 = __uint_as_float(w[e] << 16), h1 = __uint_as_float(w[e] & 0xFFFF0000u);
-              const float l0 = __uint_as_float(wl[e] << 16), l1 = __uint_as_float(wl[e] & 0xFFFF0000u);
-              a = fmaf(h0 + l0, h0 + l0, a);
-              a = fmaf(h1 + l1, h1 + l1, a);
-              alo = fmaf(l0, l0, alo);
-              alo = fmaf(l1, l1, alo);
-            }
-          }
-        }
-        a += __shfl_xor_sync(0xffffffffu, a, 1);
-        a += __shfl_xor_sync(0xffffffffu, a, 2);
-        alo += __shfl_xor_sync(0xffffffffu, alo, 1);
-        alo += __shfl_xor_sync(0xffffffffu, alo, 2);
+        float a, alo;
+        quad_row_norms(p, static_cast<int64_t>(tile) * BM + rit0 + 8 * h, q, a, alo);
         if (q == 0) ctrl->x2[rit0 + 8 * h] = a;
         xlo[h] = alo;
       }
     };
-    auto init_band = [&](auto (&sc)[2], float (&xlo)[2]) {
+    auto init_band = [&](auto (&sc)[2], float (&xlo)[2], const float* x2s) {
       const bool euclid = p.metric != VQB_METRIC_COSINE;
       const float cmax = __ldg(p.cmax + CMAX_NORM);
       const float cres = __ldg(p.cmax + CMAX_RES);
@@ -357,7 +381,7 @@
       __syncwarp();
 #pragma unroll
       for (int h = 0; h < 2; ++h) {
-        const float x2 = ctrl->x2[rit0 + 8 * h];
+        const float x2 = x2s[rit0 + 8 * h];
         const float xn = sqrtf(x2);
         const float xc = xn * cmax;
         xlo[h] = p.n_a == 2 ? sqrtf(xlo[h]) * 1.0001f : 0.f;
@@ -366,90 +390,65 @@
                    (euclid ? 0x1p-22f * (x2 + cmax * cmax) + 1e-8f : 1e-30f));
       }
     };
-    for (int t = 0, tile = static_cast<int>(blockIdx.x); tile < p.num_row_tiles; ++t, tile += static_cast<int>(gridDim.x)) {
-      typename std::conditional<WN == 128, ScanReg, ScanState<16>>::type sc[2];
-      ScanQueue<16> sq[2];
-
-      float xlo[2] = {0.f, 0.f};
-      for (int ct = 0; ct < p.num_code_steps; ++ct) {
-        const bool last_ct = ct == p.num_code_steps - 1;
-        if (WN == 256 && ct == 0) {
-          row_norms(tile, xlo);
-          init_band(sc, xlo);
-        }
-        if (gap0 >= 0) w_gap += PROF_CLOCK() - gap0;
-        { const long long c0 = PROF_CLOCK(); mbar_wait(smem_u32(&ctrl->b_full[stage]), ph); w_full += PROF_CLOCK() - c0; }
-        wgmma_fence();
-        const uint64_t sd = wgmma_desc_sw32(seed_base + (gstep % p.n_seed) * STEP_SEED_BYTES);
-        if constexpr (WN == 128) wgmma_m64n128k16_bf16_rs_set(acc, bias_a, sd);
-        else wgmma_m64n256k16_bf16_ss_set(acc, wgmma_desc_sw32(smem_u32(StepLocals<256>::bias_ones())), sd);
-        int kb = 0, ps = 0;
-        int pend_stage = -1, pend_sub = -1;
-        for (int i = 0; i < n_items; ++i) {
-          const int aplane = (ps == 2) ? 1 : 0;
-          const int sub = aplane * p.KB + kb;
-          if (ct == 0 && !stream_a) { const long long c0 = PROF_CLOCK(); mbar_wait(smem_u32(&ctrl->a_full[sub]), t & 1); w_afull += PROF_CLOCK() - c0; }
-          if (i > 0) { const long long c0 = PROF_CLOCK(); mbar_wait(smem_u32(&ctrl->b_full[stage]), ph); w_full += PROF_CLOCK() - c0; }
-          const uint32_t st_addr = b_base + stage * stage_stride;
-          const uint32_t a_addr = (stream_a ? st_addr : a_base + sub * A_SUB_BYTES) + a_row_off;
-          const uint64_t ad = wgmma_desc_sw128(a_addr);
-          const uint64_t bd = wgmma_desc_sw128(st_addr + a_stage_bytes);
-          fence_regs(acc);
-          wgmma_fence();
-#pragma unroll
-          for (int k = 0; k < 8; k += 2) {
-            if constexpr (WN == 128) wgmma_m64n128k16_bf16(acc, ad + k, bd + k);
-            else wgmma_m64n256k16_bf16(acc, ad + k, bd + k);
-          }
-          wgmma_commit();
-          if (i == n_items - 1) gap0 = PROF_CLOCK();
-          wgmma_wait<1>();
-          fence_regs(acc);
-          if (pend_stage >= 0) release(pend_stage, pend_sub);
-          const bool last_use = last_ct && !stream_a && (aplane == 1 ? ps == 2 : ps == 1);
-          pend_stage = stage;
-          pend_sub = last_use ? sub : -1;
-          if (++stage == n_ring) { stage = 0; ph ^= 1; }
-          if (++ps == p.n_passes) { ps = 0; ++kb; }
-        }
-        if (WN == 128 && ct == 0) row_norms(tile, xlo);
-        wgmma_wait<0>();
-        fence_regs(acc);
-        release(pend_stage, pend_sub);
-        ++gstep;
-        if ((ct + 1) * WN > p.Kpad) {
-#pragma unroll
-          for (int j = 0; j < WN / 8; ++j)
-#pragma unroll
-            for (int b = 0; b < 2; ++b)
-              if (ct * WN + 8 * j + 2 * q + b >= p.Kpad) { acc[4 * j + b] = -3.0e38f; acc[4 * j + 2 + b] = -3.0e38f; }
-        }
-
-        if (WN == 128 && ct == 0) {
-          init_band(sc, xlo);
-        } else if (ct > 0) {
-#pragma unroll
-          for (int h = 0; h < 2; ++h) {
-            float m = sc[h].t1;
-            m = fmaxf(m, __shfl_xor_sync(0xffffffffu, m, 1));
-            m = fmaxf(m, __shfl_xor_sync(0xffffffffu, m, 2));
-            sc[h].raise(m);
-          }
-        }
-#pragma unroll
-        for (int g = 0; g < WN / 64; ++g) {
-#pragma unroll
-          for (int h = 0; h < 2; ++h) {
-            uint32_t r[16];
-#pragma unroll
-            for (int e = 0; e < 16; ++e) r[e] = __float_as_uint(acc[4 * (8 * g + (e >> 1)) + 2 * h + (e & 1)]);
-            if constexpr (WN == 128) sc[h].template scan16<true, false>(sq[h], r, ct * WN + 64 * g + 2 * q, p.mul1);
-            else sc[h].template scan16<true>(sq[h], r, ct * WN + 64 * g + 2 * q);
-          }
-        }
-      }
-
-      if (p.fo.enabled) mbar_wait(smem_u32(&ctrl->g_empty[t & 1]), ((t >> 1) & 1) ^ 1);
+    auto begin_step = [&](float (&acc)[64]) {
+      if (gap0 >= 0) w_gap += PROF_CLOCK() - gap0;
+      { const long long c0 = PROF_CLOCK(); mbar_wait(smem_u32(&ctrl->b_full[stage]), ph); w_full += PROF_CLOCK() - c0; }
+      wgmma_fence();
+      const uint64_t sd = wgmma_desc_sw32(seed_base + (gstep % p.n_seed) * SEED_BYTES);
+      if constexpr (PIPE) wgmma_m64n128k16_bf16_ss_set(acc, wgmma_desc_sw32(smem_u32(StepLocals<true>::bias_ones())), sd);
+      else wgmma_m64n128k16_bf16_rs_set(acc, bias_a, sd);
+      kb = 0;
+      ps = 0;
+    };
+    auto issue_item = [&](float (&acc)[64], int t, bool first_ct, bool last_ct, bool first_item) {
+      const int aplane = (ps == 2) ? 1 : 0;
+      const int sub = aplane * p.KB + kb;
+      if (first_ct && !stream_a) { const long long c0 = PROF_CLOCK(); mbar_wait(smem_u32(&ctrl->a_full[sub]), t & 1); w_afull += PROF_CLOCK() - c0; }
+      if (!first_item) { const long long c0 = PROF_CLOCK(); mbar_wait(smem_u32(&ctrl->b_full[stage]), ph); w_full += PROF_CLOCK() - c0; }
+      const uint32_t st_addr = b_base + stage * stage_stride;
+      const uint32_t a_addr = (stream_a ? st_addr : a_base + sub * A_SUB_BYTES) + a_row_off;
+      const uint64_t ad = wgmma_desc_sw128(a_addr);
+      const uint64_t bd = wgmma_desc_sw128(st_addr + a_stage_bytes);
+      fence_regs(acc);
+      wgmma_fence();
+#pragma unroll
+      for (int k = 0; k < 8; k += 2) wgmma_m64n128k16_bf16(acc, ad + k, bd + k);
+      wgmma_commit();
+      const bool last_item = kb == p.KB - 1 && ps == p.n_passes - 1;
+      if (last_item) gap0 = PROF_CLOCK();
+      wgmma_wait<1>();
+      fence_regs(acc);
+      if (pend_stage >= 0) release(pend_stage, pend_sub);
+      const bool last_use = last_ct && !stream_a && (aplane == 1 ? ps == 2 : ps == 1);
+      pend_stage = stage;
+      pend_sub = last_use ? sub : -1;
+      if (++stage == n_ring) { stage = 0; ph ^= 1; }
+      if (++ps == p.n_passes) { ps = 0; ++kb; }
+    };
+    auto scan_group = [&](auto (&sc)[2], ScanQueue<16> (&sq)[2], const float (&acc)[64], int ct, int g) {
+#pragma unroll
+      for (int h = 0; h < 2; ++h) {
+        uint32_t r[16];
+#pragma unroll
+        for (int e = 0; e < 16; ++e) r[e] = __float_as_uint(acc[4 * (8 * g + (e >> 1)) + 2 * h + (e & 1)]);
+        if constexpr (PIPE) sc[h].template scan16<true>(sq[h], r, ct * WN + 64 * g + 2 * q);
+        else sc[h].template scan16<true, false>(sq[h], r, ct * WN + 64 * g + 2 * q, p.mul1);
+      }
+    };
+    auto raise_quad = [&](auto (&sc)[2]) {
+#pragma unroll
+      for (int h = 0; h < 2; ++h) {
+        float m = sc[h].t1;
+        m = fmaxf(m, __shfl_xor_sync(0xffffffffu, m, 1));
+        m = fmaxf(m, __shfl_xor_sync(0xffffffffu, m, 2));
+        sc[h].raise(m);
+      }
+    };
+    auto merge_tile = [&](auto (&sc)[2], ScanQueue<16> (&sq)[2], int t, int tile, const float* x2s) {
+      const long long m0 = PROF_CLOCK();
+      if (PIPE || p.fo.enabled) mbar_wait(smem_u32(&ctrl->g_empty[t & 1]), ((t >> 1) & 1) ^ 1);
+      const long long m1 = PROF_CLOCK();
+      w_gempty += m1 - m0;
 #pragma unroll
       for (int h = 0; h < 2; ++h) {
         const int rit = rit0 + 8 * h;
@@ -466,7 +465,7 @@
           const bool live = row < p.N && (p.row_mask == nullptr || __ldg(p.row_mask + row) != 0);
           bool exact_loss = false;
           if (TAIL >= 1 && p.fo.loss_sum && live && n < 2) {
-            float d2 = ctrl->x2[rit] - 2.f * best;
+            float d2 = x2s[rit] - 2.f * best;
             if (p.metric == VQB_METRIC_COSINE) d2 += __ldg(p.cnorm2 + i0);
             exact_loss = !(d2 >= 0x1p14f * st.W);
             if (!exact_loss) locals.loss() += d2;
@@ -496,7 +495,82 @@
         }
         __syncwarp();
       }
-      if (p.fo.enabled && lane == 0) mbar_arrive(smem_u32(&ctrl->g_full[t & 1]));
+      if ((PIPE || p.fo.enabled) && lane == 0) mbar_arrive(smem_u32(&ctrl->g_full[t & 1]));
+      w_merge += PROF_CLOCK() - m1;
+    };
+    for (int t = 0, tile = static_cast<int>(blockIdx.x); tile < p.num_row_tiles; ++t, tile += static_cast<int>(gridDim.x)) {
+      float xlo[2] = {0.f, 0.f};
+      ScanQueue<16> sq[2];
+      if constexpr (PIPE) {
+        ScanState<16> sc[2];
+        const float* nb = StepLocals<true>::norms(t & 1);
+        {
+          const long long c0 = PROF_CLOCK();
+          mbar_wait(smem_u32(&ctrl->n_full[t & 1]), (t >> 1) & 1);
+          xlo[0] = nb[BM + rit0];
+          xlo[1] = nb[BM + rit0 + 8];
+          init_band(sc, xlo, nb);
+          w_tile += PROF_CLOCK() - c0;
+        }
+        for (int ct = 0; ct < p.num_code_steps; ct += 2) {
+          const bool first_ct = ct == 0, last_ct = ct + 2 == p.num_code_steps;
+          begin_step(accA);
+          issue_item(accA, t, first_ct, false, true);
+          fence_regs(accB);
+          if (!first_ct) { raise_quad(sc); scan_group(sc, sq, accB, ct - 1, 0); }
+          issue_item(accA, t, first_ct, false, false);
+          if (!first_ct) scan_group(sc, sq, accB, ct - 1, 1);
+          for (int i = 2; i < p.KB * p.n_passes; ++i) issue_item(accA, t, first_ct, false, false);
+          ++gstep;
+          begin_step(accB);
+          issue_item(accB, t, false, last_ct, true);
+          fence_regs(accA);
+          raise_quad(sc);
+          scan_group(sc, sq, accA, ct, 0);
+          issue_item(accB, t, false, last_ct, false);
+          scan_group(sc, sq, accA, ct, 1);
+          for (int i = 2; i < p.KB * p.n_passes; ++i) issue_item(accB, t, false, last_ct, false);
+          ++gstep;
+        }
+        wgmma_wait<0>();
+        fence_regs(accB);
+        release(pend_stage, pend_sub);
+        pend_stage = -1;
+        raise_quad(sc);
+        scan_group(sc, sq, accB, p.num_code_steps - 1, 0);
+        scan_group(sc, sq, accB, p.num_code_steps - 1, 1);
+        merge_tile(sc, sq, t, tile, nb);
+      } else {
+        ScanReg sc[2];
+        for (int ct = 0; ct < p.num_code_steps; ++ct) {
+          const bool last_ct = ct == p.num_code_steps - 1;
+          begin_step(accA);
+          for (int i = 0; i < p.KB * p.n_passes; ++i) issue_item(accA, t, ct == 0, last_ct, i == 0);
+          if (ct == 0) row_norms(tile, xlo);
+          wgmma_wait<0>();
+          fence_regs(accA);
+          release(pend_stage, pend_sub);
+          pend_stage = -1;
+          ++gstep;
+          if ((ct + 1) * WN > p.Kpad) {
+#pragma unroll
+            for (int j = 0; j < WN / 8; ++j)
+#pragma unroll
+              for (int b = 0; b < 2; ++b)
+                if (ct * WN + 8 * j + 2 * q + b >= p.Kpad) { accA[4 * j + b] = -3.0e38f; accA[4 * j + 2 + b] = -3.0e38f; }
+          }
+          if (ct == 0) {
+            const long long c0 = PROF_CLOCK();
+            init_band(sc, xlo, ctrl->x2);
+            w_tile += PROF_CLOCK() - c0;
+          } else {
+            raise_quad(sc);
+          }
+          scan_group(sc, sq, accA, ct, 0);
+          scan_group(sc, sq, accA, ct, 1);
+        }
+        merge_tile(sc, sq, t, tile, ctrl->x2);
+      }
     }
     if (TAIL >= 1 && p.fo.loss_sum) {
       const double w = warp_sum(static_cast<double>(locals.loss()));
@@ -507,6 +581,9 @@
       p.prof[blockIdx.x * 16 + 3] = PROF_CLOCK() - cstart;
       p.prof[blockIdx.x * 16 + 4] = w_gap;
       p.prof[blockIdx.x * 16 + 5] = w_afull;
+      p.prof[blockIdx.x * 16 + 7] = w_tile;
+      p.prof[blockIdx.x * 16 + 8] = w_merge;
+      p.prof[blockIdx.x * 16 + 9] = w_gempty;
     }
   }
 }
@@ -570,15 +647,8 @@
   return VQB_OK;
 }
 
-static bool wide_step(const AssignPlan& pl, int Kpad, int* n_seed, int* smem_bytes) {
-  if (pl.stream_a || pl.n_stages % 2 != 0 || Kpad <= BN_STAGE) return false;
-  const int ring = pl.n_stages / 2;
-  const int seeds = (ring + pl.n_items - 1) / pl.n_items;
-  const int bytes = pl.smem_bytes - pl.n_seed * SEED_BYTES + seeds * 2 * SEED_BYTES;
-  if (bytes + WIDE_STATIC_SMEM > SMEM_LIMIT) return false;
-  *n_seed = seeds;
-  *smem_bytes = bytes;
-  return true;
+static bool pipelined_step(const AssignPlan& pl, int Kpad) {
+  return !pl.stream_a && pl.n_stages % 2 == 0 && Kpad % (2 * BN_STAGE) == 0 && pl.smem_bytes + PIPE_STATIC_SMEM <= SMEM_LIMIT;
 }
 
 }
@@ -646,11 +716,9 @@
   p.Kpad = vqb_padded_codes(K);
   p.n_a = n_a; p.n_passes = n_passes; p.KB = plan.KB;
   p.num_row_tiles = static_cast<int>((N + BM - 1) / BM);
-  int smem_bytes = plan.smem_bytes;
   p.n_seed = plan.n_seed;
-  const bool wide = wide_step(plan, p.Kpad, &p.n_seed, &smem_bytes);
-  const int WN = wide ? 256 : 128;
-  p.num_code_steps = (p.Kpad + WN - 1) / WN;
+  const bool pipe = pipelined_step(plan, p.Kpad);
+  p.num_code_steps = (p.Kpad + BN_STAGE - 1) / BN_STAGE;
   p.margin_rel = margin_rel;
   p.cmax = cmax; p.idx = idx; p.idx_prov = idx_prov; p.hist = hist; p.hist_shift = hist_shift; p.flagged = flagged; p.flag_count = flag_count; p.dbg_best = dbg_best;
   p.row_mask = row_mask;
@@ -670,33 +738,34 @@
   CUtensorMap tmA, tmB, tmS;
   rc = make_map(&tmA, a_planes, D, N, n_a, BK, BM, CU_TENSOR_MAP_SWIZZLE_128B);
   if (rc) return rc;
-  rc = make_map(&tmB, b_planes, D, p.Kpad, 2, BK, WN, CU_TENSOR_MAP_SWIZZLE_128B);
+  rc = make_map(&tmB, b_planes, D, p.Kpad, 2, BK, BN_STAGE, CU_TENSOR_MAP_SWIZZLE_128B);
   if (rc) return rc;
-  rc = make_map(&tmS, bext, 16, p.Kpad, 1, 16, WN, CU_TENSOR_MAP_SWIZZLE_32B);
+  rc = make_map(&tmS, bext, 16, p.Kpad, 1, 16, BN_STAGE, CU_TENSOR_MAP_SWIZZLE_32B);
   if (rc) return rc;
 
   static bool attr_set = false;
   if (!attr_set) {
     void (*const kernels[6])(CUtensorMap, CUtensorMap, CUtensorMap, AssignParams) = {
-        vq_assign_kernel<0, 128>, vq_assign_kernel<1, 128>, vq_assign_kernel<2, 128>,
-        vq_assign_kernel<0, 256>, vq_assign_kernel<1, 256>, vq_assign_kernel<2, 256>};
+        vq_assign_kernel<0, false>, vq_assign_kernel<1, false>, vq_assign_kernel<2, false>,
+        vq_assign_kernel<0, true>, vq_assign_kernel<1, true>, vq_assign_kernel<2, true>};
     for (int i = 0; i < 6; ++i) {
-      const int dyn = i < 3 ? SMEM_LIMIT : SMEM_LIMIT - WIDE_STATIC_SMEM;
+      const int dyn = i < 3 ? SMEM_LIMIT : SMEM_LIMIT - PIPE_STATIC_SMEM;
       const cudaError_t e = cudaFuncSetAttribute(kernels[i], cudaFuncAttributeMaxDynamicSharedMemorySize, dyn);
       if (e != cudaSuccess) return static_cast<int>(e);
     }
     attr_set = true;
   }
   const int grid = p.num_row_tiles < num_sms() ? p.num_row_tiles : num_sms();
+  const int smem_bytes = plan.smem_bytes;
   cudaStream_t s = static_cast<cudaStream_t>(stream);
-  if (wide) {
-    if (p.copy_mode) vq_assign_kernel<1, 256><<<grid, NUM_THREADS, smem_bytes, s>>>(tmA, tmB, tmS, p);
-    else if (p.resid_mode) vq_assign_kernel<2, 256><<<grid, NUM_THREADS, smem_bytes, s>>>(tmA, tmB, tmS, p);
-    else vq_assign_kernel<0, 256><<<grid, NUM_THREADS, smem_bytes, s>>>(tmA, tmB, tmS, p);
+  if (pipe) {
+    if (p.copy_mode) vq_assign_kernel<1, true><<<grid, NUM_THREADS, smem_bytes, s>>>(tmA, tmB, tmS, p);
+    else if (p.resid_mode) vq_assign_kernel<2, true><<<grid, NUM_THREADS, smem_bytes, s>>>(tmA, tmB, tmS, p);
+    else vq_assign_kernel<0, true><<<grid, NUM_THREADS, smem_bytes, s>>>(tmA, tmB, tmS, p);
   } else {
-    if (p.copy_mode) vq_assign_kernel<1, 128><<<grid, NUM_THREADS, smem_bytes, s>>>(tmA, tmB, tmS, p);
-    else if (p.resid_mode) vq_assign_kernel<2, 128><<<grid, NUM_THREADS, smem_bytes, s>>>(tmA, tmB, tmS, p);
-    else vq_assign_kernel<0, 128><<<grid, NUM_THREADS, smem_bytes, s>>>(tmA, tmB, tmS, p);
+    if (p.copy_mode) vq_assign_kernel<1, false><<<grid, NUM_THREADS, smem_bytes, s>>>(tmA, tmB, tmS, p);
+    else if (p.resid_mode) vq_assign_kernel<2, false><<<grid, NUM_THREADS, smem_bytes, s>>>(tmA, tmB, tmS, p);
+    else vq_assign_kernel<0, false><<<grid, NUM_THREADS, smem_bytes, s>>>(tmA, tmB, tmS, p);
   }
   return static_cast<int>(cudaGetLastError());
 }
```

After: 406.3 million (median of 6 runs). 7.0% higher.
